# kepengxu/RealCamNet

Hardware: AMD Instinct MI355X
Metric: megapixels/sec RAW->sRGB at 4K (higher is better)
Workload: dtype bf16; 1 GPU; cfg3: 3840x2160 Bayer mosaic -> unshuffle+pad16 -> LiteISPNet_GFM_LSC_GMA -> sRGB 3840x2160, 8 frames/GPU, bf16 storage / fp32 accumulate; frames_per_gpu=8, global_frames=8, parallelism=frame-shard x1, collective=none

## Files before the change

### include/realcam_hip.h

```cpp
#ifndef REALCAM_HIP_H
#define REALCAM_HIP_H

#include <stddef.h>
#include <stdint.h>

#ifdef __cplusplus
extern "C" {
#endif

#define RC_ABI_VERSION 15

typedef enum rc_status {
    RC_OK = 0,
    RC_ERR_INVALID = -1,
    RC_ERR_HIP = -2,
    RC_ERR_UNSUPPORTED = -3
} rc_status;

typedef enum rc_dtype { RC_F32 = 0, RC_BF16 = 1, RC_U16 = 2 ,
                        RC_F16 = 3  } rc_dtype;

typedef enum rc_act { RC_ACT_NONE = 0, RC_ACT_RELU = 1, RC_ACT_LEAKY = 2 ,
                      RC_ACT_GELU = 3 ,
                      RC_ACT_RELU_POST = 4  } rc_act;

typedef enum rc_out_mode {
    RC_OUT_NHWC = 0,
    RC_OUT_PIXEL_SHUFFLE2 = 1,
    RC_OUT_NCHW = 2,
    RC_OUT_PIXEL_SHUFFLE2_NCHW = 3,
    RC_OUT_NHWC_DWT = 4
} rc_out_mode;

int rc_abi_version(void);
const char* rc_last_error(void);
const char* rc_build_info(void);
int rc_device_arch(char* buf, size_t buflen);

int rc_bayer_unshuffle(const void* d_mosaic, int in_dtype, void* d_packed, int out_dtype,
                       int batch, int h, int w, int hp, int wp, void* stream);

int rc_raw_ingest(const void* d_mosaic, int in_dtype, void* d_packed, void* d_cond, int out_dtype, int batch, int h, int w,
                  int hp, int wp, int cond_h, int cond_w, float black_level, float white_level, void* stream);

typedef enum rc_raw_storage {
    RC_RAW_F32 = 0, RC_RAW_BF16 = 1, RC_RAW_U16 = 2, RC_RAW_F16 = 3,
    RC_RAW_U8 = 4,
    RC_RAW_MIPI10 = 5,
    RC_RAW_MIPI12 = 6
} rc_raw_storage;

typedef enum rc_cfa { RC_CFA_RGGB = 0, RC_CFA_BGGR = 1, RC_CFA_GRBG = 2, RC_CFA_GBRG = 3 } rc_cfa;

typedef struct rc_raw_format {
    int storage;
    int cfa;
    int line_bytes;
    int width;
    float black[4];
    float white;
    int reserved[4];
} rc_raw_format;
size_t rc_raw_format_size(void);

int rc_raw_ingest_fmt(const void* d_src, const rc_raw_format* fmt, void* d_packed, void* d_cond, int out_dtype, int batch, int h, int w,
                      int hp, int wp, int cond_h, int cond_w, void* stream);

int rc_rgb_encode(const void* d_src, int src_dtype, void* d_dst, int out_bits, int batch, int H, int W, int h, int w, void* stream);

typedef enum rc_yuv_layout {
    RC_YUV_NV12 = 0,
    RC_YUV_P010 = 1,
    RC_YUV_I420 = 2
} rc_yuv_layout;
typedef enum rc_yuv_matrix { RC_MATRIX_BT601 = 0, RC_MATRIX_BT709 = 1, RC_MATRIX_BT2020 = 2  } rc_yuv_matrix;
typedef enum rc_yuv_range { RC_RANGE_LIMITED = 0, RC_RANGE_FULL = 1 } rc_yuv_range;
typedef enum rc_chroma_siting { RC_SITING_LEFT = 0 ,
                                RC_SITING_CENTER = 1  } rc_chroma_siting;

#define RC_YUV_KR_KB {{0.299, 0.114}, {0.2126, 0.0722}, {0.2627, 0.0593}}

typedef struct rc_out_format {
    int layout;
    int matrix;
    int range;
    int siting;
    int pitch;
    int rows;
    int chroma_offset[2];
    int reserved[4];
} rc_out_format;
size_t rc_out_format_size(void);

size_t rc_yuv_frame_bytes(const rc_out_format* fmt, int h, int w);

int rc_yuv_encode(const void* d_src, int src_dtype, const rc_out_format* fmt, void* d_dst, int batch, int H, int W, int h, int w, void* stream);

typedef enum rc_jpeg_subsampling { RC_JPEG_420 = 0 , RC_JPEG_444 = 1  } rc_jpeg_subsampling;

typedef struct rc_jpeg_desc {
    int quality;
    int subsampling;
    int restart;
    int reserved[5];
} rc_jpeg_desc;
size_t rc_jpeg_desc_size(void);

typedef struct rc_jpeg_plan_info {
    long long header_bytes;
    long long mcu_cols, mcu_rows;
    long long intervals;
    long long capacity;
    long long scratch_bytes;
} rc_jpeg_plan_info;
// ... 423 lines not shown
```

### realcamnet_amd/LiteISP.py

```python
from __future__ import annotations

from typing import Optional, Sequence

import torch
import torch.nn as nn

from . import networks as N
from . import ops
from .groupmix import GMA_Block, SUPPORTED_DTYPES
from ._lib import RC_OUT_NCHW, RC_OUT_PIXEL_SHUFFLE2
from .jpeg import Jpeg
from .out_format import OutFormat
from .stats import Stats
from .resize import Output


def color_block(in_filters, out_filters, normalization=False):
    layers = [N.Conv2d(in_filters, out_filters, 1, stride=1, padding=0),
              nn.AvgPool2d(3, stride=2, padding=1, count_include_pad=True),
              nn.LeakyReLU(0.2)]
    if normalization:
        layers.append(nn.InstanceNorm2d(out_filters, affine=True))
    return layers

# ... 346 lines not shown
    for o in outs:
        t = y if o.warp is None else ops.warp(y, o.warp)
        t = t if o.resize is None else ops.resize(t, o.resize)
        if o.tone is not None:
            t = ops.tone_map(t, o.tone)
        if o.look is not None:
            t = ops.lut3d(t, o.look)
        if o.sharpen is not None:
            t = ops.sharpen(t, o.sharpen)
        res.append(_encode(t, _out_bits(o.format)))
    return res


class _DwtUNet(nn.Module):

    output_dtype: Optional[torch.dtype] = None
    cond_from_raw = False

    def _build(self, ch_1, ch_2, ch_3, cond_c=None, lsc=False, nf=None, n_blocks=4):
        if cond_c is not None:
            self.classifier = Color_Condition_GFM(in_channels=4, out_c=cond_c)
        self.head = N.seq(N.conv(4, ch_1, mode='C'))
        if lsc:
            self.lsc = Lens_Shading_Correction(in_channels=2, out_c=ch_1, nf=ch_1)

        def gfm(i, c):
            if cond_c is not None:
                setattr(self, f"encoder_modulation{i}", N.seq(Res_GFM(in_nc=c, chan=c, cond_c=cond_c, out_nc=c, nf=nf[i - 1])))

        gfm(1, ch_1)
        self.down1 = N.seq(N.conv(ch_1, ch_1, mode='C'), N.RCAGroup(in_channels=ch_1, out_channels=ch_1, nb=n_blocks),
                           N.conv(ch_1, ch_1, mode='C'), N.DWTForward(ch_1))
        gfm(2, ch_1 * 4)
        self.down2 = N.seq(N.conv(ch_1 * 4, ch_1, mode='C'), N.RCAGroup(in_channels=ch_1, out_channels=ch_1, nb=n_blocks),
                           N.DWTForward(ch_1))
        gfm(3, ch_1 * 4)
        self.down3 = N.seq(N.conv(ch_1 * 4, ch_2, mode='C'), N.RCAGroup(in_channels=ch_2, out_channels=ch_2, nb=n_blocks),
                           N.DWTForward(ch_2))
        gfm(4, ch_2 * 4)
        self.middle = N.seq(N.conv(ch_2 * 4, ch_3, mode='C'), N.RCAGroup(in_channels=ch_3, out_channels=ch_3, nb=n_blocks),
                            N.RCAGroup(in_channels=ch_3, out_channels=ch_3, nb=n_blocks), N.conv(ch_3, ch_2 * 4, mode='C'))
        self.up3 = N.seq(N.DWTInverse(ch_2 * 4), N.RCAGroup(in_channels=ch_2, out_channels=ch_2, nb=n_blocks),
                         N.conv(ch_2, ch_1 * 4, mode='C'))
        self.up2 = N.seq(N.DWTInverse(ch_1 * 4), N.RCAGroup(in_channels=ch_1, out_channels=ch_1, nb=n_blocks),
                         N.conv(ch_1, ch_1 * 4, mode='C'))
        self.up1 = N.seq(N.DWTInverse(ch_1 * 4), N.RCAGroup(in_channels=ch_1, out_channels=ch_1, nb=n_blocks),
                         N.conv(ch_1, ch_1, mode='C'))
        self.tail = N.seq(N.conv(ch_1, ch_1 * 4, mode='C'), nn.PixelShuffle(upscale_factor=2), N.conv(ch_1, 3, mode='C'))

    def _act_dtype(self) -> torch.dtype:
        return self.head.weight.dtype

    def _refine_d1(self, d1):
        return d1

    def _check(self, raw):
        if self.training:
            raise RuntimeError("realcamnet_amd is an inference path: call .eval() first")
        if raw.dim() != 4 or raw.shape[1] != 4:
            raise ValueError(f"raw must be (B,4,H,W), got {tuple(raw.shape)}")
        if raw.shape[2] % 8 or raw.shape[3] % 8:
            raise ValueError(f"packed RAW H,W must be multiples of 8 (3 Haar levels), got {raw.shape[2]}x{raw.shape[3]}; "
                             "use forward_mosaic()/pad_to_multiple_of_16 for other sizes")

    def _front(self, a, cond, coord_nhwc):
        def head():
            if not hasattr(self, "lsc"):
                return self.head._nhwc(a)
            h = ops.lsc_chain(self.lsc, coord_nhwc, self.head, a)
            return h if h is not None else self.head._nhwc(a, mul_plus1=self.lsc._nhwc(coord_nhwc))

        if not hasattr(self, "classifier"):
            return head(), None
        cond = ops._req(cond, "cond")
        vec, h = ops.fork_join(lambda: self.classifier._vec(cond), head, [cond])
        return h, vec

    def _trunk(self, h, vec, crop_hw=None):
        mod = (lambda i, t: getattr(self, f"encoder_modulation{i}")._nhwc((t, vec))[0]) if vec is not None else (lambda i, t: t)
        h = mod(1, h)
        d1 = self._refine_d1(self.down1._nhwc(h))
        d2 = self.down2._nhwc(mod(2, d1))
        d3 = self.down3._nhwc(mod(3, d2))
        m = self.middle._nhwc(mod(4, d3), residual=d3)
        u3 = self.up3._nhwc(m, residual=d2)
        u2 = self.up2._nhwc(u3, residual=d1)
        u1 = self.up1._nhwc(u2, residual=h)
        if ops.tail_fold_ok(u1, self.tail[0], self.tail[2]):
            return ops.tail_fold(u1, self.tail[0], self.tail[2], crop_hw=crop_hw, out_dtype=self.output_dtype)
        t = self.tail[0]._nhwc(u1, out_mode=RC_OUT_PIXEL_SHUFFLE2)
        return self.tail[2]._nhwc(t, out_mode=RC_OUT_NCHW, crop_hw=crop_hw, out_dtype=self.output_dtype)

    def forward(self, x: Sequence[torch.Tensor]):
        raw = x if isinstance(x, torch.Tensor) else x[0]
        self._check(raw)
        dt = self._act_dtype()
        coord_nhwc = None
        if hasattr(self, "lsc"):
            coord = x[2]
            if coord.shape[0] != raw.shape[0] or coord.shape[1] != 2 or coord.shape[2:] != raw.shape[2:]:
                raise ValueError(f"coord must be (B,2,H,W) matching raw, got {tuple(coord.shape)}")
            coord_nhwc = ops.to_nhwc(coord, dtype=dt)
        cond = (raw if self.cond_from_raw else x[1]) if hasattr(self, "classifier") else None
        h, vec = self._front(ops.to_nhwc(raw, dtype=dt), cond, coord_nhwc)
        return self._trunk(h, vec)

    def forward_mosaic(self, mosaic, cond=None, coord=None, pad_to: int = 16, black_level: float = 0.0, white_level: float = 1.0,
                       cond_hw=(256, 256), raw_format=None, out_format=None, outputs=None):
        if self.training:
            raise RuntimeError("realcamnet_amd is an inference path: call .eval() first")
        bits = _out_bits(out_format)
        dt = self._act_dtype()
        mh, mw = _mosaic_hw(mosaic, raw_format)
        outs = _plan_outputs(outputs, out_format, (mh, mw))
        a, cond = _ingest(self, mosaic, cond, dt, pad_to, black_level, white_level, cond_hw, raw_format)
        b, hp, wp, _ = a.shape
        co = None
        if hasattr(self, "lsc"):
            if coord is None or coord.shape[-2:] != (mh // 2, mw // 2):
                raise ValueError("coord must be at packed resolution (h, w)")
            co = ops.to_nhwc(coord, dtype=dt, pad_hw=(hp, wp))
        if hasattr(self, "classifier") and self.cond_from_raw:
            cond = ops.to_nchw(a)
        h, vec = self._front(a, cond, co)
        return _emit(self._trunk(h, vec, crop_hw=(mh, mw)), bits, outs)


class LiteISPNet(_DwtUNet):

    def __init__(self):
        super().__init__()
        self._build(64, 128, 128)


class LiteISPNet_GFM_LSC(_DwtUNet):

    def __init__(self):
        super().__init__()
        self._build(48, 128, 128, cond_c=32, lsc=True, nf=(48, 48, 48, 128))


class LiteISPNet_LSC(_DwtUNet):

    def __init__(self):
        super().__init__()
        self._build(48, 128, 128, lsc=True)


class LiteISPNet_GFM(_DwtUNet):

    def __init__(self):
        super().__init__()
        self._build(64, 128, 128, cond_c=64, nf=(64, 64, 64, 128))


class LiteISPNet_GFMresize(_DwtUNet):
    cond_from_raw = True

    def __init__(self):
        super().__init__()
        self._build(64, 128, 128, cond_c=32, nf=(128, 256, 256, 512))


class _StridedUNet(nn.Module):

    output_dtype: Optional[torch.dtype] = None

    cond_from_raw = False
    coord_in_intro = False
    skips = True
# ... 270 lines not shown
```

### realcamnet_amd/_lib.py

```python
from __future__ import annotations

import ctypes as C
import os
import re
from pathlib import Path

PKG = Path(__file__).resolve().parent
LIB_PATH = Path(os.environ["RC_HIP_LIB"]) if os.environ.get("RC_HIP_LIB") else PKG / "librealcam_hip.so"
HEADER = PKG.parent / "include" / "realcam_hip.h"

RC_F32, RC_BF16, RC_U16, RC_F16 = 0, 1, 2, 3
RC_ACT_NONE, RC_ACT_RELU, RC_ACT_LEAKY, RC_ACT_GELU, RC_ACT_RELU_POST = 0, 1, 2, 3, 4
RC_OUT_NHWC, RC_OUT_PIXEL_SHUFFLE2, RC_OUT_NCHW, RC_OUT_PIXEL_SHUFFLE2_NCHW, RC_OUT_NHWC_DWT = 0, 1, 2, 3, 4
ABI_VERSION = 15
RC_RAW_F32, RC_RAW_BF16, RC_RAW_U16, RC_RAW_F16, RC_RAW_U8, RC_RAW_MIPI10, RC_RAW_MIPI12 = 0, 1, 2, 3, 4, 5, 6
RC_CFA_RGGB, RC_CFA_BGGR, RC_CFA_GRBG, RC_CFA_GBRG = 0, 1, 2, 3
RC_YUV_NV12, RC_YUV_P010, RC_YUV_I420 = 0, 1, 2
RC_MATRIX_BT601, RC_MATRIX_BT709, RC_MATRIX_BT2020 = 0, 1, 2
RC_RANGE_LIMITED, RC_RANGE_FULL = 0, 1
RC_SITING_LEFT, RC_SITING_CENTER = 0, 1
RC_JPEG_420, RC_JPEG_444 = 0, 1
RC_FILTER_AREA, RC_FILTER_BILINEAR = 0, 1
RC_RESIZE_MAX_TAPS, RC_RESIZE_MAX_RATIO = 20, 8
RC_LUT3D_MIN_SIZE, RC_LUT3D_MAX_SIZE = 2, 65
RC_WARP_BILINEAR, RC_WARP_BICUBIC = 0, 1
RC_WARP_CLAMP, RC_WARP_CONSTANT = 0, 1
RC_WARP_MIN_CELL_LOG2, RC_WARP_MAX_CELL_LOG2, RC_WARP_MAX_DIM = 3, 6, 1 << 23
RC_STATS_MAX_GRID, RC_STATS_SLOTS = 64, 8
RC_TONE_MAX_GRID, RC_TONE_BINS = 16, 256
RC_DEFECT_HOT, RC_DEFECT_COLD = 1, 2
RC_CALIB_GAINS, RC_CALIB_CLIP, RC_CALIB_MAX_KNOTS = 1, 2, 16
RC_HDR_MOTION = 1
RC_TNR_RESET, RC_TNR_GAIN = 1, 2
RC_QUAD_REMOSAIC, RC_QUAD_BIN = 0, 1


class ConvDesc(C.Structure):
    _fields_ = [
        ("batch", C.c_int32), ("height", C.c_int32), ("width", C.c_int32),
        ("cin", C.c_int32), ("cout", C.c_int32), ("ksize", C.c_int32),
        ("dtype", C.c_int32),
        ("in0", C.c_void_p), ("in1", C.c_void_p), ("in_gate", C.c_void_p), ("in_store", C.c_void_p),
        ("wpacked", C.c_void_p), ("bias", C.c_void_p),
        ("film_scale", C.c_void_p), ("film_shift", C.c_void_p),
        ("act", C.c_int32), ("act_slope", C.c_float),
        ("mul_plus1", C.c_void_p), ("residual", C.c_void_p),
        ("out", C.c_void_p), ("out_mode", C.c_int32), ("out_dtype", C.c_int32),
        ("out_h", C.c_int32), ("out_w", C.c_int32),
        ("chan_sums", C.c_void_p),
        ("src_h", C.c_int32), ("src_w", C.c_int32),
        ("out_scale", C.c_void_p),
        ("chan_sums_slots", C.c_int32), ("cout_tile", C.c_int32),
        ("algo", C.c_int32),
    ]


class ConvPairDesc(C.Structure):
    _fields_ = [
        ("batch", C.c_int32), ("height", C.c_int32), ("width", C.c_int32), ("channels", C.c_int32),
        ("dtype", C.c_int32),
        ("in0", C.c_void_p), ("in1", C.c_void_p), ("in_gate", C.c_void_p), ("in_store", C.c_void_p),
        ("w1", C.c_void_p), ("b1", C.c_void_p),
        ("film_scale", C.c_void_p), ("film_shift", C.c_void_p),
        ("act1", C.c_int32), ("act1_slope", C.c_float),
        ("w2", C.c_void_p), ("b2", C.c_void_p),
        ("residual", C.c_void_p), ("out", C.c_void_p), ("chan_sums", C.c_void_p),
    ]


class RawFormatDesc(C.Structure):
    _fields_ = [
        ("storage", C.c_int32), ("cfa", C.c_int32), ("line_bytes", C.c_int32), ("width", C.c_int32),
        ("black", C.c_float * 4), ("white", C.c_float), ("reserved", C.c_int32 * 4),
    ]


class OutFormatDesc(C.Structure):
    _fields_ = [
        ("layout", C.c_int32), ("matrix", C.c_int32), ("range", C.c_int32), ("siting", C.c_int32),
        ("pitch", C.c_int32), ("rows", C.c_int32), ("chroma_offset", C.c_int32 * 2), ("reserved", C.c_int32 * 4),
    ]


class JpegDesc(C.Structure):
    _fields_ = [("quality", C.c_int32), ("subsampling", C.c_int32), ("restart", C.c_int32), ("reserved", C.c_int32 * 5)]


class JpegPlanInfo(C.Structure):
    _fields_ = [("header_bytes", C.c_longlong), ("mcu_cols", C.c_longlong), ("mcu_rows", C.c_longlong), ("intervals", C.c_longlong),
                ("capacity", C.c_longlong), ("scratch_bytes", C.c_longlong)]


class StatsDesc(C.Structure):
    _fields_ = [
        ("roi", C.c_int32 * 4), ("grid", C.c_int32 * 2), ("bits", C.c_int32), ("matrix", C.c_int32), ("dark", C.c_int32), ("clip", C.c_int32),
        ("reserved", C.c_int32 * 4),
# ... 257 lines not shown
```

### realcamnet_amd/csrc/conv.hip

```cpp
#include <mutex>
#include <vector>

#include "conv32_kernel.hpp"

namespace rc {

struct ConvPlan {
    int ck = 0, nt = 0, unit = 0, upt = 0, nu = 0, steps = 0;
    int n_chunks = 0, n_ct = 0, cout_packed = 0;
    int m32 = 0;
};

static int g_persist_on = 1;
extern int g_dw3_seg16;
extern int g_dec_lds;
extern int g_wmsa_mfma;
extern int g_pw_grid_cap;
static int g_pss = 0;
static int g_poison = 0;
static int g_thin = 2;
static int g_auto = 1;
static int g_sums_compact = 1;
static int g_conv32 = 0;

// ... 235 lines not shown
    if (std::string(key) == "pair_impl") { g_pair_impl = value < 0 || value > 2 ? 0 : value; return RC_OK; }
    if (std::string(key) == "dec_lds") { g_dec_lds = value != 0; return RC_OK; }
    if (std::string(key) == "dw3_seg16") { g_dw3_seg16 = value != 0; return RC_OK; }
    if (std::string(key) == "wmsa_mfma") { g_wmsa_mfma = value != 0; return RC_OK; }
    if (std::string(key) == "pss") { g_pss = value != 0; return RC_OK; }
    if (std::string(key) == "sums_compact") { g_sums_compact = value != 0; return RC_OK; }
    if (std::string(key) == "persist_auto") { g_auto = value < 0 ? 0 : (value > 2 ? 2 : value); return RC_OK; }
    if (std::string(key) == "thin") { g_thin = value < 0 ? 0 : (value > 2 ? 2 : value); return RC_OK; }
    if (std::string(key) == "lds_poison") { g_poison = value != 0; return RC_OK; }
    if (std::string(key) == "conv32") { g_conv32 = value < 0 ? 0 : (value > 4 ? 4 : value); return RC_OK; }
    if (std::string(key) == "wino_nnt") { wino_set_nnt(value); return RC_OK; }
    if (std::string(key) == "pw_grid_cap") { g_pw_grid_cap = value <= 0 || value > (1 << 22) ? (1 << 22) : value; return RC_OK; }
    return fail(RC_ERR_INVALID, std::string("rc_debug_set: unknown key ") + key);
}

int rc_debug_get(const char* key) {
    if (key == nullptr) return -1;
    if (std::string(key) == "persist") return g_persist_on;
    if (std::string(key) == "conv32") return g_conv32;
    if (std::string(key) == "conv_flags") return g_dbg_flags;
    if (std::string(key) == "pss") return g_pss;
    if (std::string(key) == "sums_compact") return g_sums_compact;
    if (std::string(key) == "persist_auto") return g_auto;
    if (std::string(key) == "thin") return g_thin;
    if (std::string(key) == "lds_poison") return g_poison;
    if (std::string(key) == "wino_nnt") return wino_get_nnt();
    if (std::string(key) == "pw_grid_cap") return g_pw_grid_cap;
    return -1;
}

int rc_debug_set_ptr(const char* key, void* p) {
    RC_REQUIRE(key != nullptr, "rc_debug_set_ptr: null key");
    if (std::string(key) == "conv_phase_timing") { g_dbg_ptr = static_cast<long long*>(p); return RC_OK; }
    return fail(RC_ERR_INVALID, std::string("rc_debug_set_ptr: unknown key ") + key);
}

int rc_prof_enable(int on) {
    std::lock_guard<std::mutex> lk(g_prof_mu);
    for (auto& r : g_prof) { (void)hipEventDestroy(r.e0); (void)hipEventDestroy(r.e1); }
    g_prof.clear();
    g_prof_on = on != 0;
    return RC_OK;
}

int rc_prof_collect(int64_t* n_launches, double* total_ms, double* total_flops) {
    std::lock_guard<std::mutex> lk(g_prof_mu);
    double ms = 0.0, fl = 0.0;
    for (auto& r : g_prof) {
        RC_HIP_CHECK(hipEventSynchronize(r.e1));
        float t = 0.f;
        RC_HIP_CHECK(hipEventElapsedTime(&t, r.e0, r.e1));
        ms += t; fl += r.flops;
    }
    if (n_launches) *n_launches = (int64_t)g_prof.size();
    if (total_ms) *total_ms = ms;
    if (total_flops) *total_flops = fl;
    return RC_OK;
}

int rc_prof_collect_rows(rc_prof_row* rows, int max_rows, int* n_rows) {
    RC_REQUIRE(rows != nullptr && n_rows != nullptr && max_rows >= 1, "rc_prof_collect_rows: bad arguments");
    std::lock_guard<std::mutex> lk(g_prof_mu);
    int n = 0;
    for (auto& r : g_prof) {
        RC_HIP_CHECK(hipEventSynchronize(r.e1));
        float t = 0.f;
        RC_HIP_CHECK(hipEventElapsedTime(&t, r.e0, r.e1));
        int i = 0;
        while (i < n && !(rows[i].cin == r.cin && rows[i].cout == r.cout && rows[i].ksize == r.ksize)) ++i;
        if (i == n) {
            if (n == max_rows) continue;
            rows[n] = rc_prof_row{r.cin, r.cout, r.ksize, 0, 0.0, 0.0, 0.0};
            ++n;
        }
        rows[i].launches += 1; rows[i].ms += t; rows[i].flops += r.flops; rows[i].bytes += r.bytes;
    }
    *n_rows = n;
    return RC_OK;
}

static int conv_build_args(const rc_conv_desc* d, ConvPlan& p, ConvArgs& a, size_t& es_out) {
    RC_REQUIRE(d != nullptr, "rc_conv2d: null desc");
    const bool dwt = d->out_mode == RC_OUT_NHWC_DWT;
    RC_REQUIRE(make_plan(d->cin, d->cout, d->ksize, d->dtype, dwt ? (int)RC_OUT_NHWC : d->out_mode, &p, d->cout_tile), "rc_conv2d: unsupported cin/cout/ksize/dtype/cout_tile");
    RC_REQUIRE(d->batch >= 1 && d->height >= 1 && d->width >= 1, "rc_conv2d: empty tensor");
    RC_REQUIRE(d->batch <= 65535, "rc_conv2d: batch > 65535");
    RC_REQUIRE(d->in0 && d->wpacked && d->out, "rc_conv2d: null in0/wpacked/out");
    RC_REQUIRE(d->out_mode >= RC_OUT_NHWC && d->out_mode <= RC_OUT_NHWC_DWT, "rc_conv2d: bad out_mode");
    if (dwt) {
        RC_REQUIRE(d->height % 2 == 0 && d->width % 2 == 0, "rc_conv2d: RC_OUT_NHWC_DWT needs even height and width");
        RC_REQUIRE(d->out_dtype == d->dtype && reinterpret_cast<uintptr_t>(d->out) % 16 == 0, "rc_conv2d: RC_OUT_NHWC_DWT: out_dtype must equal dtype, out 16-byte aligned");
        RC_REQUIRE(!d->mul_plus1 && !d->film_scale && !d->out_scale && !d->chan_sums && !d->in_gate && !d->in1 && !d->in_store && !d->src_h && !d->src_w && !d->cout_tile,
                   "rc_conv2d: RC_OUT_NHWC_DWT excludes mul_plus1 / film / out_scale / chan_sums / gated input / src_h / cout_tile");
        if (d->dtype == RC_F32 || d->ksize != 3 || p.m32 || !(d->act == RC_ACT_NONE || ((d->act == RC_ACT_RELU || d->act == RC_ACT_LEAKY) && !d->residual)))
            return fail(RC_ERR_UNSUPPORTED, "rc_conv2d: RC_OUT_NHWC_DWT is a bf16 / fp16 3x3 form with act NONE / RELU / LEAKY, or act NONE + residual");
    }
    RC_REQUIRE(d->act >= RC_ACT_NONE && d->act <= RC_ACT_RELU_POST, "rc_conv2d: bad act");
    RC_REQUIRE(d->act != RC_ACT_RELU_POST || (d->residual != nullptr && d->mul_plus1 == nullptr && d->film_scale == nullptr && d->chan_sums == nullptr),
               "rc_conv2d: RC_ACT_RELU_POST is relu(conv + residual): needs residual, excludes film / mul_plus1 / chan_sums");
    if (d->in_gate) RC_REQUIRE(d->in1 != nullptr, "rc_conv2d: in_gate needs in1 (the skip tensor)");
    RC_REQUIRE((d->film_scale == nullptr) == (d->film_shift == nullptr), "rc_conv2d: film_scale/film_shift must come together");
    const bool full_tiles = d->cout == p.cout_packed;
    if (d->mul_plus1 || d->residual)
        RC_REQUIRE((full_tiles || d->cout % 4 == 0) && (d->out_mode == RC_OUT_NHWC || (dwt && !d->mul_plus1)), "rc_conv2d: mul_plus1/residual need cout % 4 == 0 and RC_OUT_NHWC (residual: or RC_OUT_NHWC_DWT)");
    if (d->chan_sums) RC_REQUIRE(d->out_mode == RC_OUT_NHWC, "rc_conv2d: chan_sums needs RC_OUT_NHWC");
    if (d->out_scale) {
        RC_REQUIRE(d->out_mode == RC_OUT_NHWC && !p.m32, "rc_conv2d: out_scale needs RC_OUT_NHWC and a layer outside the 32x32x16 forms");
        RC_REQUIRE(reinterpret_cast<uintptr_t>(d->out_scale) % 4 == 0, "rc_conv2d: out_scale must be 4-byte aligned");
    }
    const size_t es = dtype_size(d->dtype);
    const int planar16 = d->dtype == RC_F16 ? RC_F16 : RC_BF16;
    if (dwt) {
    } else if (d->out_mode == RC_OUT_NHWC) {
        RC_REQUIRE(d->out_dtype == d->dtype, "rc_conv2d: out_dtype must equal dtype for RC_OUT_NHWC");
        RC_REQUIRE(!full_tiles || (d->cout * es) % 8 == 0, "rc_conv2d: cout*elem_size must be a multiple of 8 bytes for RC_OUT_NHWC");
        RC_REQUIRE(reinterpret_cast<uintptr_t>(d->out) % 16 == 0, "rc_conv2d: out must be 16-byte aligned");
        if (p.nt == 4 && d->dtype != RC_F32) RC_REQUIRE(d->cout % 8 == 0, "rc_conv2d: cout % 8");
    } else if (d->out_mode == RC_OUT_PIXEL_SHUFFLE2) {
        RC_REQUIRE(d->out_dtype == d->dtype, "rc_conv2d: out_dtype must equal dtype for RC_OUT_PIXEL_SHUFFLE2");
        RC_REQUIRE(full_tiles && ((d->cout / 4) * es) % 8 == 0, "rc_conv2d: pixel-shuffle store needs (cout/4)*elem_size % 8 == 0");
        RC_REQUIRE(!d->film_scale, "rc_conv2d: film not supported with pixel-shuffle store");
        RC_REQUIRE(reinterpret_cast<uintptr_t>(d->out) % 16 == 0, "rc_conv2d: out must be 16-byte aligned");
    } else if (d->out_mode == RC_OUT_PIXEL_SHUFFLE2_NCHW) {
        RC_REQUIRE(d->out_h >= 1 && d->out_h <= 2 * d->height && d->out_w >= 1 && d->out_w <= 2 * d->width, "rc_conv2d: bad pixel-shuffle NCHW crop");
        RC_REQUIRE(d->out_dtype == RC_F32 || d->out_dtype == planar16, "rc_conv2d: bad out_dtype");
        RC_REQUIRE(!d->chan_sums, "rc_conv2d: chan_sums needs RC_OUT_NHWC");
        RC_REQUIRE((double)d->out_h * d->out_w * (d->cout / 4) * 4.0 < 2147483647.0, "rc_conv2d: one output image must be < 2 GiB");
    } else {
        RC_REQUIRE(d->out_h >= 1 && d->out_h <= d->height && d->out_w >= 1 && d->out_w <= d->width, "rc_conv2d: bad NCHW crop");
        RC_REQUIRE(d->out_dtype == RC_F32 || d->out_dtype == planar16, "rc_conv2d: bad out_dtype");
    }
    {
        const double lim = 2147483647.0;
        RC_REQUIRE((double)d->height * d->width * d->cin * es < lim, "rc_conv2d: one input image must be < 2 GiB");
        RC_REQUIRE((double)d->height * d->width * d->cout * 4.0 < lim, "rc_conv2d: one output image must be < 2 GiB");
    }
    const bool fold = d->src_h != 0 || d->src_w != 0;
    if (fold) {
        RC_REQUIRE(d->ksize == 2 && d->cin % 4 == 0 && (d->cin / 4) % p.ck == 0, "rc_conv2d: src_h/src_w need ksize 2 and cin / 4 a whole number of Cin chunks");
        RC_REQUIRE(d->src_h >= 1 && d->src_w >= 1 && d->height == (d->src_h + 1) / 2 && d->width == (d->src_w + 1) / 2,
                   "rc_conv2d: height/width must be ceil(src_h / 2), ceil(src_w / 2)");
        RC_REQUIRE(d->in_gate == nullptr && d->in1 == nullptr && d->in_store == nullptr, "rc_conv2d: src_h/src_w exclude the gated input");
        RC_REQUIRE(reinterpret_cast<uintptr_t>(d->in0) % 16 == 0, "rc_conv2d: src_h/src_w need a 16-byte aligned in0 (the scalar staging path does not gather)");
        RC_REQUIRE((double)d->src_h * d->src_w * (d->cin / 4) * es < 2147483647.0, "rc_conv2d: one input image must be < 2 GiB");
    }
    if (d->residual) RC_REQUIRE(reinterpret_cast<uintptr_t>(d->residual) % 16 == 0, "rc_conv2d: residual must be 16-byte aligned");
    if (d->mul_plus1) RC_REQUIRE(reinterpret_cast<uintptr_t>(d->mul_plus1) % 16 == 0, "rc_conv2d: mul_plus1 must be 16-byte aligned");

    a = ConvArgs{};
    a.batch = d->batch; a.H = d->height; a.W = d->width; a.cin = d->cin; a.cout = d->cout;
    a.n_chunks = p.n_chunks; a.n_ct = p.n_ct;
    a.tiles_x = ceil_div(d->width, kTW); a.tiles_y = ceil_div(d->height, kTH);
    if (p.m32) RC_REQUIRE(!d->film_scale || (reinterpret_cast<uintptr_t>(d->film_scale) % 16 == 0 && reinterpret_cast<uintptr_t>(d->film_shift) % 16 == 0),
                          "rc_conv2d: film vectors must be 16-byte aligned");
    auto aligned16 = [](const void* q) { return q == nullptr || reinterpret_cast<uintptr_t>(q) % 16 == 0; };
    a.cin_vec_ok = (d->cin % p.unit == 0) && aligned16(d->in0) && aligned16(d->in1) && aligned16(d->in_store) &&
                   (d->in_gate == nullptr || reinterpret_cast<uintptr_t>(d->in_gate) % 4 == 0);
    a.cin_chunk_ok = d->cin % p.ck == 0;
    a.fold2 = fold ? 1 : 0; a.src_H = d->src_h; a.src_W = d->src_w; a.cfold = d->cin / 4;
    a.in0 = d->in0; a.in1 = d->in1; a.in_gate = d->in_gate; a.in_store = d->in_store;
    a.wpacked = d->wpacked; a.bias = d->bias;
    a.film_scale = d->film_scale; a.film_shift = d->film_shift;
    a.act = d->act; a.act_slope = d->act_slope;
    a.mul_plus1 = d->mul_plus1; a.residual = d->residual; a.out_scale = d->out_scale;
    a.out = d->out; a.out_mode = d->out_mode; a.out_dtype = d->out_dtype; a.out_h = d->out_h; a.out_w = d->out_w;
    a.chan_sums = d->chan_sums; a.cout_packed = p.cout_packed;
    a.sum_slots = d->chan_sums_slots > 0 ? d->chan_sums_slots : 4 * ceil_div(d->height, kTH) * ceil_div(d->width, kTW);
    a.sums_compact = 0; a.query = nullptr; a.sums_compact_ok = g_sums_compact;
    {
        int key = (d->act == RC_ACT_RELU ? 1 : 0) | (d->act == RC_ACT_LEAKY ? 2 : 0) | (d->film_scale ? 4 : 0) |
                  (d->mul_plus1 ? 8 : 0) | (d->residual ? 16 : 0) | (d->chan_sums ? 32 : 0) | (d->out_scale ? 64 : 0);
        bool fast = full_tiles && d->out_mode != RC_OUT_NCHW && d->out_mode != RC_OUT_PIXEL_SHUFFLE2_NCHW && d->act != RC_ACT_GELU && d->act != RC_ACT_RELU_POST;
        if (d->act == RC_ACT_LEAKY) fast = fast && d->act_slope >= 0.f && d->act_slope <= 1.f;
        if (d->film_scale)
            fast = fast && d->cout % 4 == 0 && reinterpret_cast<uintptr_t>(d->film_scale) % 16 == 0 && reinterpret_cast<uintptr_t>(d->film_shift) % 16 == 0;
        if (d->out_scale) fast = fast && d->cout % 4 == 0 && reinterpret_cast<uintptr_t>(d->out_scale) % 16 == 0;
        switch (key) { case 0: case 1: case 2: case 16: case 32: case 8: case 6: case 33: case 34: case 80: break; default: fast = false; }
        a.ep_key = fast ? key : -1;
        a.pss = g_pss && d->out_mode == RC_OUT_PIXEL_SHUFFLE2 && !p.m32 && p.n_chunks == 1 && p.n_ct == 4 && d->cout == 4 * 16 * p.nt &&
                d->dtype == RC_BF16 && d->in_gate == nullptr && fast && (key == 0 || key == 1 || key == 2);
    }
    {
        const int num_cus = device_cu_count();
        a.num_cus = num_cus;
        a.persist_ok = g_persist_on;
        a.auto_impl = g_auto;
        a.thin = g_thin;
        a.dbg = g_dbg_ptr;
        a.dbg_flags = g_dbg_flags;
        a.td = make_tile_decode(a.tiles_x, a.tiles_y, kBandRows);
        a.td_wsm = make_tile_decode(a.tiles_x, (a.H + kWsmTH - 1) / kWsmTH, kBandRows);
        a.div_n_ct = make_magic(a.n_ct);
    }
    es_out = es;
    return RC_OK;
// ... 44 lines not shown
```

### realcamnet_amd/csrc/conv_kernel.hpp

```cpp
#pragma once
#include "common.hpp"

namespace rc {

struct MagicDiv { unsigned m, sh; };
inline MagicDiv make_magic(int d) {
    if (d <= 1) return MagicDiv{0u, 0u};
    int L = 0;
    while ((2 << L) <= d) ++L;
    const unsigned long long m = ((1ull << (31 + L)) + (unsigned long long)d - 1) / (unsigned long long)d;
    return MagicDiv{(unsigned)m, (unsigned)(L - 1)};
}
__device__ __forceinline__ int magic_div(int n, const MagicDiv& d) {
    return d.m ? (int)(__umulhi((unsigned)n, d.m) >> d.sh) : n;
}
struct TileDecode { MagicDiv sp_total, band, last_rows; };
inline TileDecode make_tile_decode(int tiles_x, int tiles_y, int band_rows) {
    return TileDecode{make_magic(tiles_x * tiles_y), make_magic(band_rows * tiles_x), make_magic(tiles_y % band_rows ? tiles_y % band_rows : 1)};
}

struct ConvArgs {
    int batch, H, W, cin, cout;
    int n_chunks, n_ct, tiles_x, tiles_y;
    int cin_vec_ok;
// ... 822 lines not shown
            if constexpr ((F & EP_SUMS) != 0) {
#pragma unroll
                for (int e = 0; e < NV; ++e) run[e] += valid ? v[e] : 0.f;
            }
            const int oo = (valid && !(a.dbg_flags & 1)) ? (((gy + p) * a.W + gx) * a.cout + jbase) * ES : kOOB;
            buf_store_row<T, NV, PK_RELU>(r_out, oo, v);
        }
        if constexpr ((F & EP_SUMS) != 0) {
            if (flush) {
                write_chan_sums(a, b, slot, n, jbase, run, false);
#pragma unroll
                for (int e = 0; e < NV; ++e) run[e] = 0.f;
            }
        }
    }

    template <int F>
    __device__ static __forceinline__ void epilogue_dwt(const ConvArgs& a, int b, int y0, int x0, int tid, f32x4 (&acc)[4][NT], char* st,
                                                        const unsigned (&rp)[(F & EP_RES) ? 4 : 1][(F & EP_RES) ? NV / 2 : 1]) {
        static_assert(ES == 2 && NV % 4 == 0 && (F == 0 || F == EP_RELU || F == EP_LEAKY || F == EP_RES), "bf16; plain / ReLU / LeakyReLU / + residual");
        typedef float f32x2 __attribute__((ext_vector_type(2)));
        const int lane = tid & 63, wave = tid >> 6, q = lane >> 4, n = lane & 15;
        constexpr int REC = Cfg::COUT_TILE * 2 + 8, ROW = kTW * REC;
        const float inf = __builtin_inff();
#pragma unroll
        for (int pt = 0; pt < 4; ++pt) {
            float v[NV];
#pragma unroll
            for (int nt = 0; nt < NT; ++nt)
#pragma unroll
                for (int r = 0; r < 4; ++r) v[nt * 4 + r] = acc[pt][nt][r];
            if constexpr ((F & EP_RELU) != 0) {
#pragma unroll
                for (int e = 0; e < NV; ++e) v[e] = __builtin_amdgcn_fmed3f(v[e], 0.f, inf);
            }
            if constexpr ((F & EP_LEAKY) != 0) {
#pragma unroll
                for (int e = 0; e < NV; ++e) v[e] = __builtin_amdgcn_fmed3f(v[e], v[e] * a.act_slope, inf);
            }
            if constexpr ((F & EP_RES) != 0) {
#pragma unroll
                for (int i = 0; i < NV / 2; ++i) {
                    v[2 * i] += lo16<T>(rp[pt][i]);
                    v[2 * i + 1] += hi16<T>(rp[pt][i]);
                }
            }
            char* dst = st + (pt >> 1) * ROW + (16 * (pt & 1) + n) * REC + q * (NV * 2);
#pragma unroll
            for (int i = 0; i < NV / 4; ++i)
                *reinterpret_cast<uint2*>(dst + 8 * i) = make_uint2(pack16x2<T>(v[4 * i], v[4 * i + 1]), pack16x2<T>(v[4 * i + 2], v[4 * i + 3]));
        }
        __builtin_amdgcn_fence(__ATOMIC_RELEASE, "wavefront");
        __builtin_amdgcn_wave_barrier();
        f32x2 in[4][NV / 2];
        const char* src = st + (2 * n) * REC + q * (NV * 2);
#pragma unroll
        for (int t = 0; t < 4; ++t)
#pragma unroll
            for (int i = 0; i < NV / 4; ++i) {
                const uint2 w = *reinterpret_cast<const uint2*>(src + (t >> 1) * ROW + (t & 1) * REC + 8 * i);
                in[t][2 * i] = f32x2{lo16<T>(w.x), hi16<T>(w.x)} * 0.5f;
                in[t][2 * i + 1] = f32x2{lo16<T>(w.y), hi16<T>(w.y)} * 0.5f;
            }
        __builtin_amdgcn_fence(__ATOMIC_RELEASE, "wavefront");
        __builtin_amdgcn_wave_barrier();
        unsigned o[2 * NV];
#pragma unroll
        for (int p = 0; p < NV / 2; ++p) {
            const f32x2 sab = in[0][p] + in[1][p], dab = in[0][p] - in[1][p];
            const f32x2 k0 = (sab + in[2][p]) + in[3][p], k1 = (sab - in[2][p]) - in[3][p];
            const f32x2 k2 = (dab + in[2][p]) - in[3][p], k3 = (dab - in[2][p]) + in[3][p];
            o[4 * p] = pack16x2<T>(k0.x, k1.x); o[4 * p + 1] = pack16x2<T>(k2.x, k3.x);
            o[4 * p + 2] = pack16x2<T>(k0.y, k1.y); o[4 * p + 3] = pack16x2<T>(k2.y, k3.y);
        }
        const int Hh = a.H >> 1, Wh = a.W >> 1, oy = (y0 >> 1) + wave, ox = (x0 >> 1) + n;
        const size_t img_out = (size_t)a.H * a.W * a.cout;
        const __amdgpu_buffer_rsrc_t r_out = make_rsrc(static_cast<T*>(a.out) + (size_t)b * img_out, (unsigned)(img_out * ES));
        const int oo = (oy < Hh && ox < Wh && !(a.dbg_flags & 1)) ? ((oy * Wh + ox) * (4 * a.cout) + 4 * q * NV) * ES : kOOB;
#pragma unroll
        for (int i = 0; i < NV / 2; ++i)
            __builtin_amdgcn_raw_buffer_store_b128(u32x4_t{o[4 * i], o[4 * i + 1], o[4 * i + 2], o[4 * i + 3]}, r_out, oo, 16 * i, 0);
    }

    __device__ static __forceinline__ void epilogue_generic(const ConvArgs& a, int b, int y0, int x0, int sp, int ct, int tid,
                                                            f32x4 (&acc)[4][NT]) {
        const int lane = tid & 63, wave = tid >> 6, q = lane >> 4, n = lane & 15;
        const int jbase = ct * Cfg::COUT_TILE + q * NV;
        float fs[NV], ft[NV];
        const bool film = a.film_scale != nullptr;
        if (film) {
#pragma unroll
            for (int e = 0; e < NV; ++e) {
                const bool in = jbase + e < a.cout;
                fs[e] = in ? a.film_scale[(size_t)b * a.cout + jbase + e] : 0.f;
                ft[e] = in ? a.film_shift[(size_t)b * a.cout + jbase + e] : 0.f;
            }
        }
        const int gy_w = y0 + 2 * wave, gx_l = x0 + n;
        float csum[NV];
#pragma unroll
        for (int e = 0; e < NV; ++e) csum[e] = 0.f;

        const size_t img_out = (size_t)a.H * a.W * a.cout;
        const unsigned img_bytes_out = (unsigned)(img_out * ES);
        __amdgpu_buffer_rsrc_t r_out;
        if (a.out_mode == RC_OUT_NCHW || a.out_mode == RC_OUT_PIXEL_SHUFFLE2_NCHW) {
            const size_t plane = (size_t)a.out_h * a.out_w;
            const int osz = a.out_dtype == RC_F32 ? 4 : 2;
            const int planes = a.out_mode == RC_OUT_NCHW ? a.cout : a.cout >> 2;
            r_out = make_rsrc(static_cast<char*>(a.out) + (size_t)b * planes * plane * osz, (unsigned)(planes * plane * osz));
        } else {
            r_out = make_rsrc(static_cast<T*>(a.out) + (size_t)b * img_out, img_bytes_out);
        }
        const bool full = a.cout == a.cout_packed;

#pragma unroll
        for (int pt = 0; pt < 4; ++pt) {
            const int gy = gy_w + (pt >> 1);
            const int gx = gx_l + (pt & 1) * 16;
            const bool valid = gy < a.H && gx < a.W;
            float v[NV];
#pragma unroll
            for (int nt = 0; nt < NT; ++nt)
#pragma unroll
                for (int r = 0; r < 4; ++r) v[nt * 4 + r] = acc[pt][nt][r];
            if (film) {
#pragma unroll
                for (int e = 0; e < NV; ++e) v[e] = v[e] * fs[e] + ft[e] + v[e];
            }
            if (a.act == RC_ACT_RELU) {
#pragma unroll
                for (int e = 0; e < NV; ++e) v[e] = __builtin_amdgcn_fmed3f(v[e], 0.f, __builtin_inff());
            } else if (a.act == RC_ACT_LEAKY) {
#pragma unroll
                for (int e = 0; e < NV; ++e) v[e] = v[e] > 0.f ? v[e] : v[e] * a.act_slope;
            } else if (a.act == RC_ACT_GELU) {
#pragma unroll
                for (int e = 0; e < NV; ++e) v[e] = gelu_erf_f32(v[e]);
            }
            const int pix_off = valid ? ((gy * a.W + gx) * a.cout + jbase) * ES : kOOB;
            if (a.mul_plus1 != nullptr) {
                float m[NV];
                const __amdgpu_buffer_rsrc_t r_mul = make_rsrc(static_cast<const T*>(a.mul_plus1) + (size_t)b * img_out, img_bytes_out);
                buf_load_row<T, NV>(r_mul, pix_off, m);
#pragma unroll
                for (int e = 0; e < NV; ++e) v[e] = v[e] * (m[e] + 1.f);
            }
            if (a.out_scale != nullptr) {
#pragma unroll
                for (int e = 0; e < NV; ++e) v[e] *= (jbase + e < a.cout) ? a.out_scale[(size_t)b * a.cout + jbase + e] : 0.f;
            }
            if (a.residual != nullptr) {
                float m[NV];
                const __amdgpu_buffer_rsrc_t r_res = make_rsrc(static_cast<const T*>(a.residual) + (size_t)b * img_out, img_bytes_out);
                buf_load_row<T, NV>(r_res, pix_off, m);
#pragma unroll
                for (int e = 0; e < NV; ++e) v[e] += m[e];
                if (a.act == RC_ACT_RELU_POST) {
#pragma unroll
                    for (int e = 0; e < NV; ++e) v[e] = __builtin_amdgcn_fmed3f(v[e], 0.f, __builtin_inff());
                }
            }
            if (a.chan_sums != nullptr) {
#pragma unroll
                for (int e = 0; e < NV; ++e) csum[e] += valid ? v[e] : 0.f;
            }
// ... 58 lines not shown

template <class Cfg, bool GATED, bool FAST>
__global__ __launch_bounds__(kThreads, 2) void conv_mfma_kernel(const ConvArgs a) {
    using D = ConvDev<Cfg>;
    using T = typename Cfg::elem;
    constexpr int NT = Cfg::NT, STEPS = Cfg::STEPS, G = Cfg::G, NSUB = Cfg::NSUB, NV = 4 * NT;

    extern __shared__ __attribute__((aligned(16))) char smem[];
    char* s_w = smem;
    char* s_in = smem + Cfg::W_BYTES;

    const int tid = threadIdx.x, lane = tid & 63, wave = tid >> 6;
    const int q = lane >> 4, n = lane & 15;
    const int ct = blockIdx.x % a.n_ct;
    const int sp = blockIdx.x / a.n_ct;
    const int tx = sp % a.tiles_x, ty = sp / a.tiles_x;
    const int b = blockIdx.y;
    const int y0 = ty * kTH, x0 = tx * kTW;

    typename D::LaneOff lo;
    D::lane_offsets(q, lo);
    const int lane_x = ((2 * wave) * D::TWH + n) * D::SPIX;
    const int lane_w = lane * 16;

    f32x4 acc[4][NT];
#pragma unroll
    for (int nt = 0; nt < NT; ++nt) {
        f32x4 bv = f32x4{0.f, 0.f, 0.f, 0.f};
        if (a.bias) {
            const float4 t4 = *reinterpret_cast<const float4*>(a.bias + ct * Cfg::COUT_TILE + q * NV + nt * 4);
            bv = f32x4{t4.x, t4.y, t4.z, t4.w};
        }
#pragma unroll
        for (int pt = 0; pt < 4; ++pt) acc[pt][nt] = bv;
    }

    ConvArgs aa = a;
    if (ct != 0) aa.in_store = nullptr;
    const typename D::TileSrc ts = D::tile_src(aa, b, y0, x0);
    typename D::TileOffs to;
    D::tile_offsets(aa, tid, to);
    const char* wbase = static_cast<const char*>(a.wpacked) + (size_t)ct * a.n_chunks * Cfg::CHUNK_W_BYTES;

    for (int chunk = 0; chunk < a.n_chunks; ++chunk) {
        if (chunk > 0) __syncthreads();
        const char* wchunk = wbase + (size_t)chunk * Cfg::CHUNK_W_BYTES;
        D::dma_weights(wchunk, s_w, (STEPS < G ? STEPS : G) * NT, wave, lane_w);
        if (a.cin_vec_ok) {
            uint4 r0[D::NI], r1[GATED ? D::NI : 1];
            float gv[GATED ? D::UNIT : 1];
            D::template load_tile<GATED>(aa, ts, to, b, chunk, tid, r0, r1, gv);
            D::template commit_tile<GATED>(aa, ts, to, chunk, tid, r0, r1, gv, s_in);
        } else {
            D::stage_tile_scalar(aa, b, y0, x0, chunk, tid, s_in, static_cast<T*>(aa.in_store));
        }
        __syncthreads();
        D::template mma_steps<0, G, 0>(s_in, s_w, lane_x, lane_w, q, lo, acc);
        if constexpr (NSUB > 1) {
            __syncthreads();
            D::dma_weights(wchunk + (size_t)G * NT * 1024, s_w, ((STEPS - G) < G ? (STEPS - G) : G) * NT, wave, lane_w);
            __syncthreads();
            D::template mma_steps<G, G, G>(s_in, s_w, lane_x, lane_w, q, lo, acc);
        }
        if constexpr (NSUB > 2) {
            __syncthreads();
            D::dma_weights(wchunk + (size_t)2 * G * NT * 1024, s_w, ((STEPS - 2 * G) < G ? (STEPS - 2 * G) : G) * NT, wave, lane_w);
            __syncthreads();
            D::template mma_steps<2 * G, G, 2 * G>(s_in, s_w, lane_x, lane_w, q, lo, acc);
        }
        static_assert(NSUB <= 3, "add another weight sub-stage");
    }
    D::template epilogue<FAST>(a, b, y0, x0, sp, ct, tid, acc);
}

constexpr int kPersistMaxCout = 512;
template <class Cfg>
constexpr int persist_bias_slots() { return Cfg::KS == 5 ? 64 : kPersistMaxCout; }
template <class Cfg>
constexpr int persist_lds_bytes_c() { return Cfg::IN_BYTES + (int)Cfg::CHUNK_W_BYTES + persist_bias_slots<Cfg>() * 4; }

template <class Cfg>
constexpr int persist_blocks_per_cu() { return Cfg::NT <= 2 && persist_lds_bytes_c<Cfg>() * 3 <= 160 * 1024 ? 3 : 2; }

template <class Cfg, bool GATED, bool FAST>
__global__ __launch_bounds__(kThreads, persist_blocks_per_cu<Cfg>()) void conv_mfma_persist_kernel(const ConvArgs a) {
    using D = ConvDev<Cfg>;
    constexpr int NT = Cfg::NT, STEPS = Cfg::STEPS, NV = 4 * NT;

    const int w_copies = a.w_resident ? a.n_ct : 1;
    extern __shared__ __attribute__((aligned(16))) char smem[];
    char* s_w = smem;
    float* s_bias = reinterpret_cast<float*>(smem + w_copies * Cfg::CHUNK_W_BYTES);
    char* s_in = smem + w_copies * Cfg::CHUNK_W_BYTES + persist_bias_slots<Cfg>() * 4;

    const int tid = threadIdx.x, lane = tid & 63, wave = tid >> 6;
    const int q = lane >> 4, n = lane & 15;
    typename D::LaneOff lo;
    D::lane_offsets(q, lo);
    const int lane_x = ((2 * wave) * D::TWH + n) * D::SPIX;
    const int lane_w = lane * 16;

    const int sp_total = a.tiles_x * a.tiles_y;
    const int n_tiles = sp_total * a.batch;
    const int n_ct = a.n_ct;
    const int slots = gridDim.x >> 3;
    const int pos = (blockIdx.x & 7) * slots + (blockIdx.x >> 3);

    if (n_ct == 1 || a.w_resident) D::dma_weights(static_cast<const char*>(a.wpacked), s_w, STEPS * NT * w_copies, wave, lane_w);
    for (int i = tid; i < a.cout_packed; i += kThreads) s_bias[i] = a.bias ? a.bias[i] : 0.f;

    uint4 r0[D::NI], r1[GATED ? D::NI : 1];
    float gv[GATED ? D::UNIT : 1];
    typename D::TileOffs to;
    D::tile_offsets(a, tid, to);
    int tile = pos < n_tiles ? pos : -1;
    int b = 0, sp = 0, y0 = 0, x0 = 0;
    typename D::TileSrc ts;
    if (tile >= 0) {
        b = magic_div(tile, a.td.sp_total);
        int ty, tx;
        band_decode(tile - b * sp_total, a.tiles_x, a.tiles_y, a.td, ty, tx);
        sp = ty * a.tiles_x + tx; y0 = ty * kTH; x0 = tx * kTW;
        ts = D::tile_src(a, b, y0, x0);
        if (a.cin_vec_ok) {
            D::template load_gate<GATED>(a, b, 0, tid, gv);
            if (ts.interior) D::template load_tile_interior<GATED>(a, ts, to, 0, r0, r1);
        }
    }
    float run[NV];
#pragma unroll
    for (int e = 0; e < NV; ++e) run[e] = 0.f;
    int covered = 0;
    constexpr bool BORDER_PRE = !GATED && Cfg::KS == 3 && (NT == 3 || NT == 4) && sizeof(typename Cfg::elem) == 2;
    bool first_tile = true;
    while (tile >= 0) {
        __syncthreads();
        if (a.cin_vec_ok && !ts.interior && (!BORDER_PRE || first_tile || (a.dbg_flags & 16))) D::template load_tile_border<GATED>(a, ts, 0, tid, r0, r1);
        first_tile = false;
        if (a.cin_vec_ok) D::template commit_tile<GATED>(a, ts, to, 0, tid, r0, r1, gv, s_in);
        else D::stage_tile_scalar(a, b, y0, x0, 0, tid, s_in, static_cast<typename Cfg::elem*>(a.in_store));
        constexpr bool RUN_SUMS = FAST && sizeof(typename Cfg::elem) == 2 && NT >= 3;
        const int cb = b, csp = sp, cy0 = y0, cx0 = x0;
        const int next = tile + (int)gridDim.x;
        tile = next < n_tiles ? next : -1;
        if constexpr (RUN_SUMS) {
            const bool will_flush = tile < 0 || magic_div(tile, a.td.sp_total) != cb;
            if ((a.ep_key == D::EP_SUMS || a.ep_key == (D::EP_RELU | D::EP_SUMS)) && n_ct == 1) {
                if (!a.sums_compact) { if (!will_flush) D::zero_sum_slots(a, cb, csp, tid); }
                else if (will_flush) {
                    for (int bb = covered; bb < cb; ++bb) D::zero_slots4(a, bb, 4 * D::compact_residue(pos, bb, sp_total, (int)gridDim.x), tid);
                    covered = cb + 1;
                }
            }
        }

        for (int ct = 0; ct < n_ct; ++ct) {
            if (n_ct > 1 && !a.w_resident) {
                if (ct > 0) __syncthreads();
                D::dma_weights(static_cast<const char*>(a.wpacked) + (size_t)ct * Cfg::CHUNK_W_BYTES, s_w, STEPS * NT, wave, lane_w);
            }
            if (ct == 0 || !a.w_resident) __syncthreads();
            if (ct == n_ct - 1 && tile >= 0) {
                b = magic_div(tile, a.td.sp_total);
                int ty, tx;
                band_decode(tile - b * sp_total, a.tiles_x, a.tiles_y, a.td, ty, tx);
                sp = ty * a.tiles_x + tx; y0 = ty * kTH; x0 = tx * kTW;
                ts = D::tile_src(a, b, y0, x0);
                if (a.cin_vec_ok) {
                    D::template load_gate<GATED>(a, b, 0, tid, gv);
                    if (ts.interior) D::template load_tile_interior<GATED>(a, ts, to, 0, r0, r1);
                    else if constexpr (BORDER_PRE) { if (!(a.dbg_flags & 16)) D::template load_tile_border<GATED>(a, ts, 0, tid, r0, r1); }
                }
            }
            f32x4 acc[4][NT];
#pragma unroll
            for (int nt = 0; nt < NT; ++nt) {
                const float4 t4 = *reinterpret_cast<const float4*>(s_bias + ct * Cfg::COUT_TILE + q * NV + nt * 4);
#pragma unroll
                for (int pt = 0; pt < 4; ++pt) acc[pt][nt] = f32x4{t4.x, t4.y, t4.z, t4.w};
            }
            constexpr bool RESPRE = FAST && !GATED && sizeof(typename Cfg::elem) == 2 && NT <= 3;
            [[maybe_unused]] unsigned rpre[RESPRE ? 4 : 1][RESPRE ? D::NRH : 1];
            bool res_pre = false;
            if constexpr (RESPRE) {
                if ((a.ep_key == D::EP_RES || a.ep_key == (D::EP_GATE | D::EP_RES)) && a.out_mode == RC_OUT_NHWC) {
                    res_pre = true;
                    D::res_prefetch(a, cb, cy0, cx0, ct, tid, rpre);
                }
            }
            D::template mma_steps<0, STEPS, 0, (!GATED && NT < 5)>(s_in, a.w_resident ? s_w + ct * (int)Cfg::CHUNK_W_BYTES : s_w, lane_x, lane_w, q, lo, acc);
            if constexpr (FAST && sizeof(typename Cfg::elem) == 2) {
                const int rslot = a.sums_compact ? 4 * D::compact_residue(pos, cb, sp_total, (int)gridDim.x) : -1;
                if (RUN_SUMS && a.ep_key == D::EP_SUMS && n_ct == 1)
                    D::template epilogue_fast_impl<D::EP_SUMS, RUN_SUMS>(a, cb, cy0, cx0, csp, ct, tid, acc, run, tile < 0 || b != cb, rslot);
                else if (RUN_SUMS && a.ep_key == (D::EP_RELU | D::EP_SUMS) && n_ct == 1)
                    D::template epilogue_fast_impl<D::EP_RELU | D::EP_SUMS, RUN_SUMS>(a, cb, cy0, cx0, csp, ct, tid, acc, run, tile < 0 || b != cb, rslot);
                else if (res_pre) {
                    if constexpr (RESPRE) {
                        D::epilogue_res_pre(a, cb, cy0, cx0, ct, tid, acc, rpre, a.ep_key == (D::EP_GATE | D::EP_RES) ? a.out_scale + (size_t)cb * a.cout : nullptr);
                    }
                } else D::template epilogue<FAST>(a, cb, cy0, cx0, csp, ct, tid, acc);
            } else D::template epilogue<FAST>(a, cb, cy0, cx0, csp, ct, tid, acc);
        }
    }
    if constexpr (FAST && sizeof(typename Cfg::elem) == 2 && NT >= 3) {
        if (a.sums_compact && (a.ep_key == D::EP_SUMS || a.ep_key == (D::EP_RELU | D::EP_SUMS)) && n_ct == 1)
            for (int bb = covered; bb < a.batch; ++bb) D::zero_slots4(a, bb, 4 * D::compact_residue(pos, bb, sp_total, (int)gridDim.x), tid);
    }
}

constexpr int kWsThreads = 512;

template <class Cfg, bool GATED, bool FAST>
__global__ __launch_bounds__(kWsThreads) void conv_mfma_ws_kernel(const ConvArgs a) {
    using D = ConvDev<Cfg>;
    constexpr int NT = Cfg::NT, STEPS = Cfg::STEPS, NV = 4 * NT;

    extern __shared__ __attribute__((aligned(16))) char smem[];
    char* s_w = smem;
    float* s_bias = reinterpret_cast<float*>(smem + Cfg::CHUNK_W_BYTES);
    char* s_buf0 = smem + Cfg::CHUNK_W_BYTES + 16 * Cfg::NT * 4;
    char* s_buf1 = s_buf0 + Cfg::IN_BYTES;

    const int tid = threadIdx.x, lane = tid & 63;
    const int wave8 = __builtin_amdgcn_readfirstlane(tid >> 6);
    const bool loader = wave8 >= 4;
    const int rtid = tid & 255, wave = wave8 & 3;
    const int q = lane >> 4, n = lane & 15;

    const int sp_total = a.tiles_x * a.tiles_y;
    const int n_tiles = sp_total * a.batch;
    const int slots = gridDim.x >> 3;
    const int pos = (blockIdx.x & 7) * slots + (blockIdx.x >> 3);
    const int stride = (int)gridDim.x;
    const int my_tiles = pos < n_tiles ? (n_tiles - pos + stride - 1) / stride : 0;

    for (int kb = wave8; kb < STEPS * NT; kb += kWsThreads / 64)
        __builtin_amdgcn_global_load_lds((const __attribute__((address_space(1))) void*)(static_cast<const char*>(a.wpacked) + kb * 1024 + lane * 16),
                                         (__attribute__((address_space(3))) void*)(s_w + kb * 1024), 16, 0, 0);
    for (int i = tid; i < a.cout_packed; i += kWsThreads) s_bias[i] = a.bias ? a.bias[i] : 0.f;

    auto decode = [&](int tile, int& b, int& sp, int& y0, int& x0) {
        b = magic_div(tile, a.td.sp_total);
        int ty, tx;
        band_decode(tile - b * sp_total, a.tiles_x, a.tiles_y, a.td, ty, tx);
        sp = ty * a.tiles_x + tx; y0 = ty * kTH; x0 = tx * kTW;
    };

    if (loader) {
        uint4 r0[D::NI], r1[GATED ? D::NI : 1];
        float gv[GATED ? D::UNIT : 1];
        typename D::TileSrc ts;
        typename D::TileOffs to;
        D::tile_offsets(a, rtid, to);
        int b, sp, y0, x0;
        if (my_tiles > 0) {
            decode(pos, b, sp, y0, x0);
            ts = D::tile_src(a, b, y0, x0);
            D::template load_tile<GATED>(a, ts, to, b, 0, rtid, r0, r1, gv);
            D::template commit_tile<GATED>(a, ts, to, 0, rtid, r0, r1, gv, s_buf0);
        }
        if (my_tiles > 1) {
            decode(pos + stride, b, sp, y0, x0);
            ts = D::tile_src(a, b, y0, x0);
            D::template load_tile<GATED>(a, ts, to, b, 0, rtid, r0, r1, gv);
        }
        __syncthreads();
        const bool rec = a.dbg != nullptr && blockIdx.x == 8 && wave8 == 4 && lane == 0;
        for (int k = 0; k < my_tiles; ++k) {
            const long long tl0 = rec ? (long long)__builtin_amdgcn_s_memtime() : 0;
            if (k + 1 < my_tiles) {
                D::template commit_tile<GATED>(a, ts, to, 0, rtid, r0, r1, gv, ((k + 1) & 1) ? s_buf1 : s_buf0);
                if (k + 2 < my_tiles) {
                    decode(pos + (k + 2) * stride, b, sp, y0, x0);
// ... 128 lines not shown
        __syncthreads();
        for (int g = 0; g < my_stages; ++g) {
            const int wsoff_g = wsoff;
            dma(WA, WB, wsoff_g);
            if (g + 1 < my_stages) issue_a();
            __syncthreads();
            if (g + 1 < my_stages) {
                if (need_wa()) dma(0, WA, wsoff);
                commit_a();
            }
            __syncthreads();
        }
    } else {
        const int wave = wave12;
        typename D::LaneOff lo;
        D::lane_offsets(q, lo);
        const int lane_x = ((2 * wave) * D::TWH + n) * D::SPIX;
        const int lane_w = lane * 16;
        __syncthreads();
        int g = 0;
        for (int k = 0; k < my_units; ++k) {
            int b, ty, tx, ct0;
            decode(pos + k * stride, b, ty, tx, ct0);
            const int ty8 = 2 * ty + (wave >> 2);
            for (int ct = ct0; ct < ct0 + cts_per_unit; ++ct) {
                f32x4 acc[4][NT];
#pragma unroll
                for (int nt = 0; nt < NT; ++nt) {
                    const float4 t4 = *reinterpret_cast<const float4*>(s_bias + ct * Cfg::COUT_TILE + q * NV + nt * 4);
#pragma unroll
                    for (int pt = 0; pt < 4; ++pt) acc[pt][nt] = f32x4{t4.x, t4.y, t4.z, t4.w};
                }
                auto run_chunks = [&](auto PH, int c0, int c1) {
                    constexpr int ph = decltype(PH)::value;
                    for (int c = c0; c < c1; ++c, ++g) {
                        const char* s_in = s_in0 + (one_chunk ? (k & 1) : (g & 1)) * Cfg::IN_BYTES;
                        if constexpr (ph == 3) { if (!(a.dbg_flags & 2)) D::template mma_steps<0, SA, 0, true>(s_in, s_w, lane_x, lane_w, q, lo, acc); }
                        else if constexpr (ph == 2) D::template mma_steps<1, 1, 0, false>(s_in, s_w, lane_x, lane_w, q, lo, acc);
                        __syncthreads();
                        if constexpr ((ph & 1) != 0) { if (!(a.dbg_flags & 2)) D::template mma_steps<SA, STEPS - SA, 0, true>(s_in, s_w, lane_x, lane_w, q, lo, acc); }
                        else D::template mma_steps<3, 1, 0, false>(s_in, s_w, lane_x, lane_w, q, lo, acc);
                        if (c + 1 < n_chunks) __syncthreads();
                    }
                };
                if constexpr (FOLD_SKIP) {
                    const int cpp = D::folded(a) ? n_chunks >> 2 : 0;
                    run_chunks(std::integral_constant<int, 0>{}, 0, cpp);
                    run_chunks(std::integral_constant<int, 1>{}, cpp, 2 * cpp);
                    run_chunks(std::integral_constant<int, 2>{}, 2 * cpp, 3 * cpp);
                    run_chunks(std::integral_constant<int, 3>{}, 3 * cpp, n_chunks);
                } else {
                    run_chunks(std::integral_constant<int, 3>{}, 0, n_chunks);
                }
                if (ty8 < a.tiles_y)
                    D8::template epilogue<FAST>(a, b, ty8 * kTH, tx * kTW, ty8 * a.tiles_x + tx, ct, tid & 255, acc);
                __syncthreads();
            }
        }
    }
}

template <class Cfg8>
struct WstCfg : WsmCfg<Cfg8> {
    using B = WsmCfg<Cfg8>;
    static constexpr int SPIX = B::CK * (int)sizeof(typename B::elem);
    static constexpr int N_PIECES = B::THH * B::TWH * B::UPT;
    static constexpr int N_DMA = (N_PIECES + 63) / 64;
    static constexpr int IN_BYTES = N_DMA * 1024;
};
template <class Cfg>
constexpr int wst_form() {
    if (!(sizeof(typename Cfg::elem) == 2 && (Cfg::KS == 2 || Cfg::KS == 3) && (Cfg::UPT == 2 || Cfg::UPT == 4) && Cfg::STEPS >= 2)) return 0;
    const int w = (int)Cfg::CHUNK_W_BYTES, in = WstCfg<Cfg>::IN_BYTES, fixed = 2 * w + kPersistMaxCout * 4;
    if (w <= 20 * 1024 && fixed + 3 * in <= 160 * 1024) return 3;
    if (w <= 36 * 1024 && fixed + 2 * in <= 160 * 1024) return 2;
    return 0;
}
template <class Cfg>
constexpr int wst_lds_bytes() { return 2 * (int)Cfg::CHUNK_W_BYTES + kPersistMaxCout * 4 + (wst_form<Cfg>() == 3 ? 3 : 2) * WstCfg<Cfg>::IN_BYTES; }
template <class Cfg>
constexpr bool wst_eligible() { return wst_form<Cfg>() != 0; }
constexpr int waitcnt_vm(int n) { return (n & 15) | ((n >> 4) << 14) | 0x0F70; }

template <class Cfg8, bool FAST>
__global__ __launch_bounds__(kWsmThreads) void conv_mfma_wst_kernel(const ConvArgs a) {
#if defined(__HIP_DEVICE_COMPILE__)
    using Cfg = WstCfg<Cfg8>;
    using D = ConvDev<Cfg>;
    using D8 = ConvDev<Cfg8>;
    constexpr int NT = Cfg::NT, STEPS = Cfg::STEPS, NV = 4 * NT, WALL = (int)Cfg::CHUNK_W_BYTES, UPT = Cfg::UPT, TWH = Cfg::TWH, ES = 2;
    constexpr int N_DMA = Cfg::N_DMA, NDW = (N_DMA + 3) / 4;
    constexpr int NBUF = wst_form<Cfg8>() == 3 ? 3 : 2;
    constexpr bool FOLD_SKIP = Cfg::KS == 2 && UPT == 4 && STEPS == 4;

    extern __shared__ __attribute__((aligned(16))) char smem[];
    char* s_w = smem;
    float* s_bias = reinterpret_cast<float*>(smem + 2 * WALL);
    char* s_in0 = smem + 2 * WALL + kPersistMaxCout * 4;

    const int tid = threadIdx.x, lane = tid & 63;
    const int wave12 = __builtin_amdgcn_readfirstlane(tid >> 6);
    const bool loader = wave12 >= 8;
    const int q = lane >> 4, n = lane & 15;

    const int tiles_y = (a.H + kWsmTH - 1) / kWsmTH;
    const int sp_total = a.tiles_x * tiles_y;
    const int n_tiles = sp_total * a.batch;
    const int n_chunks = a.n_chunks, n_ct = a.n_ct;
    const bool one_chunk = n_chunks == 1;
    const int n_units = one_chunk ? n_tiles : n_tiles * n_ct;
    const int cts_per_unit = one_chunk ? n_ct : 1;
    const int slots = gridDim.x >> 3;
    const int pos = (blockIdx.x & 7) * slots + (blockIdx.x >> 3);
    const int stride = (int)gridDim.x;
    const int my_units = pos < n_units ? (n_units - pos + stride - 1) / stride : 0;
    const int my_stages = my_units * cts_per_unit * n_chunks;

    for (int i = tid; i < a.cout_packed; i += kWsmThreads) s_bias[i] = a.bias ? a.bias[i] : 0.f;

    auto decode = [&](int unit, int& b, int& ty, int& tx, int& ct0) {
        int tile = unit;
        ct0 = 0;
        if (!one_chunk) { tile = magic_div(unit, a.div_n_ct); ct0 = unit - tile * n_ct; }
        b = magic_div(tile, a.td_wsm.sp_total);
        band_decode(tile - b * sp_total, a.tiles_x, tiles_y, a.td_wsm, ty, tx);
    };

    if (loader && NBUF == 2) {
        if constexpr (NBUF == 2) {
            const int rtid = tid - kWsmCompute, w4 = wave12 - 8;
            uint4 r0[D::NI], r1[1];
            float gv[1];
            typename D::TileSrc ts;
            typename D::TileOffs to;
            D::tile_offsets(a, rtid, to);
            int k_unit = 0, cti = 0, chunk = 0, gi = 0, ct = 0;
            int b = 0, ty = 0, tx = 0, ct0 = 0;
            auto fetch = [&]() {
                if (gi < my_stages) {
                    if (chunk == 0) {
                        if (cti == 0) decode(pos + k_unit * stride, b, ty, tx, ct0);
                        ct = ct0 + cti;
                        ts = D::tile_src(a, b, ty * kWsmTH, tx * kTW);
                    }
                    const int goff = (ct * n_chunks + chunk) * WALL;
                    for (int kb = w4; kb < WALL / 1024; kb += 4)
                        __builtin_amdgcn_global_load_lds((const __attribute__((address_space(1))) void*)(static_cast<const char*>(a.wpacked) + goff + kb * 1024 + lane * 16),
                                                         (__attribute__((address_space(3))) void*)(s_w + (gi & 1) * WALL + kb * 1024), 16, 0, 0);
                    if (!one_chunk || cti == 0) {
                        D::template load_tile<false>(a, ts, to, b, chunk, rtid, r0, r1, gv);
                        D::template commit_tile<false>(a, ts, to, chunk, rtid, r0, r1, gv, s_in0 + (one_chunk ? (k_unit & 1) : (gi & 1)) * Cfg::IN_BYTES);
                    }
                }
                ++gi;
                if (++chunk == n_chunks) { chunk = 0; if (++cti == cts_per_unit) { cti = 0; ++k_unit; } }
            };
            fetch();
            __syncthreads();
            for (int g = 0; g < my_stages; ++g) {
                fetch();
                __syncthreads();
            }
        }
    } else if (loader) {
        const int w4 = wave12 - 8;
        int lc[NDW];
#pragma unroll
// ... 36 lines not shown
                    }
                }
            }
            ++gi; gb3 = gb3 == 2 ? 0 : gb3 + 1;
            if (++chunk == n_chunks) { chunk = 0; if (++cti == cts_per_unit) { cti = 0; ++k_unit; kb3 = kb3 == 2 ? 0 : kb3 + 1; } }
            return in_flight;
        };
        int wi = 0, wk = 0, wcti = 0, wchunk = 0, wct0 = 0;
        auto issue_w = [&]() {
            if (wi < my_stages) {
                if (wchunk == 0 && wcti == 0) { int b_, ty_, tx_; decode(pos + wk * stride, b_, ty_, tx_, wct0); }
                const int goff = ((wct0 + wcti) * n_chunks + wchunk) * WALL;
                int ph = 3;
                if constexpr (FOLD_SKIP) ph = D::folded(a) ? D::fold_phase(a, wchunk * Cfg::CK) : 3;
                for (int kb = w4; kb < WALL / 1024; kb += 4) {
                    if constexpr (FOLD_SKIP) {
                        const int st = kb / NT;
                        if (!(st == 3 || ph == 3 || (ph == 1 && st == 2) || (ph == 2 && st == 1))) continue;
                    }
                    __builtin_amdgcn_global_load_lds((const __attribute__((address_space(1))) void*)(static_cast<const char*>(a.wpacked) + goff + kb * 1024 + lane * 16),
                                                     (__attribute__((address_space(3))) void*)(s_w + (wi & 1) * WALL + kb * 1024), 16, 0, 0);
                }
            }
            ++wi;
            if (++wchunk == n_chunks) { wchunk = 0; if (++wcti == cts_per_unit) { wcti = 0; ++wk; } }
        };
        issue_w();
        issue();
        issue();
        __syncthreads();
        for (int g = 0; g < my_stages; ++g) {
            issue_w();
            const int nfl = issue();
            if (nfl == NDW) __builtin_amdgcn_s_waitcnt(waitcnt_vm(NDW));
            else if (NDW > 1 && nfl == NDW - 1) __builtin_amdgcn_s_waitcnt(waitcnt_vm(NDW > 1 ? NDW - 1 : 0));
            else __builtin_amdgcn_s_waitcnt(waitcnt_vm(0));
            __builtin_amdgcn_s_barrier();
        }
        __builtin_amdgcn_s_waitcnt(waitcnt_vm(0));
    } else {
        const int wave = wave12;
        typename D::LaneOff lo;
        D::lane_offsets(q, lo);
        const int lane_x = ((2 * wave) * D::TWH + n) * D::SPIX;
        const int lane_w = lane * 16;
        __syncthreads();
        int g = 0, gb3 = 0, kb3 = 0;
        for (int k = 0; k < my_units; ++k) {
            int b, ty, tx, ct0;
            decode(pos + k * stride, b, ty, tx, ct0);
            const int ty8 = 2 * ty + (wave >> 2);
            for (int ct = ct0; ct < ct0 + cts_per_unit; ++ct) {
                f32x4 acc[4][NT];
#pragma unroll
                for (int nt = 0; nt < NT; ++nt) {
                    const float4 t4 = *reinterpret_cast<const float4*>(s_bias + ct * Cfg::COUT_TILE + q * NV + nt * 4);
#pragma unroll
                    for (int pt = 0; pt < 4; ++pt) acc[pt][nt] = f32x4{t4.x, t4.y, t4.z, t4.w};
                }
                auto run_chunks = [&](auto PH, int c0, int c1) {
                    constexpr int ph = decltype(PH)::value;
                    for (int c = c0; c < c1; ++c, ++g) {
                        const char* s_in = s_in0 + (one_chunk ? kb3 : gb3) * Cfg::IN_BYTES;
                        const char* s_wg = s_w + (g & 1) * WALL;
                        if constexpr (ph == 3) D::template mma_steps<0, STEPS, 0, true>(s_in, s_wg, lane_x, lane_w, q, lo, acc);
                        else if constexpr (ph == 1) D::template mma_steps<2, 2, 0, true>(s_in, s_wg, lane_x, lane_w, q, lo, acc);
                        else {
                            if constexpr (ph == 2) D::template mma_steps<1, 1, 0, false>(s_in, s_wg, lane_x, lane_w, q, lo, acc);
                            D::template mma_steps<3, 1, 0, false>(s_in, s_wg, lane_x, lane_w, q, lo, acc);
                        }
                        gb3 = gb3 == NBUF - 1 ? 0 : gb3 + 1;
                        if (c + 1 < n_chunks) __syncthreads();
                    }
                };
                if constexpr (FOLD_SKIP) {
                    const int cpp = D::folded(a) ? n_chunks >> 2 : 0;
                    run_chunks(std::integral_constant<int, 0>{}, 0, cpp);
                    run_chunks(std::integral_constant<int, 1>{}, cpp, 2 * cpp);
                    run_chunks(std::integral_constant<int, 2>{}, 2 * cpp, 3 * cpp);
                    run_chunks(std::integral_constant<int, 3>{}, 3 * cpp, n_chunks);
                } else {
                    run_chunks(std::integral_constant<int, 3>{}, 0, n_chunks);
                }
                if (ty8 < a.tiles_y)
                    D8::template epilogue<FAST>(a, b, ty8 * kTH, tx * kTW, ty8 * a.tiles_x + tx, ct, tid & 255, acc);
                __syncthreads();
            }
            kb3 = kb3 == NBUF - 1 ? 0 : kb3 + 1;
        }
    }
#endif
}

template <class Cfg>
constexpr int pss_lds_bytes() { return (int)Cfg::CHUNK_W_BYTES + kPersistMaxCout * 4 + WsmCfg<Cfg>::IN_BYTES + kWsmTH * kTW * Cfg::COUT_TILE * 2; }

template <class Cfg8>
__global__ __launch_bounds__(kWsmThreads) void conv_mfma_pss_kernel(const ConvArgs a) {
    using Cfg = WsmCfg<Cfg8>;
    using D = ConvDev<Cfg>;
    using T = typename Cfg::elem;
    static_assert(sizeof(T) == 2, "bf16 form");
    constexpr int NT = Cfg::NT, STEPS = Cfg::STEPS, NV = 4 * NT, NH = NV / 2;
    constexpr int SA = (STEPS + 1) / 2;
    constexpr int WA = SA * NT * 1024, WB = (STEPS - SA) * NT * 1024, WALL = (int)Cfg::CHUNK_W_BYTES;
    constexpr int NWA = (WA / 16 + kThreads - 1) / kThreads, NWB = (WB / 16 + kThreads - 1) / kThreads;
    constexpr int PXB = Cfg::COUT_TILE * 2, ROWB = kTW * PXB, OUTB = kWsmTH * ROWB;
    constexpr int UPP = PXB / 16, UPR = kTW * UPP;
    constexpr int NDR = OUTB / 16 / kThreads;
    static_assert(STEPS >= 2 && WA + WB == WALL && OUTB % (16 * kThreads) == 0 && NDR % 2 == 0 && PXB % 16 == 0, "pss shapes");

    extern __shared__ __attribute__((aligned(16))) char smem[];
    char* s_w = smem;
    float* s_bias = reinterpret_cast<float*>(smem + WALL);
    char* s_in = smem + WALL + kPersistMaxCout * 4;
    char* s_out = s_in + Cfg::IN_BYTES;

    const int tid = threadIdx.x, lane = tid & 63;
    const int wave12 = __builtin_amdgcn_readfirstlane(tid >> 6);
    const bool loader = wave12 >= 8;
    const int q = lane >> 4, n = lane & 15;

    const int tiles_y = (a.H + kWsmTH - 1) / kWsmTH;
    const int sp_total = a.tiles_x * tiles_y;
    const int n_tiles = sp_total * a.batch;
    constexpr int n_ct = 4;
    const int slots = gridDim.x >> 3;
    const int pos = (blockIdx.x & 7) * slots + (blockIdx.x >> 3);
    const int stride = (int)gridDim.x;
    const int my_units = pos < n_tiles ? (n_tiles - pos + stride - 1) / stride : 0;
    const int my_stages = my_units * n_ct;
    const int cps = a.cout >> 2;

    for (int i = tid; i < a.cout_packed; i += kWsmThreads) s_bias[i] = a.bias ? a.bias[i] : 0.f;

    auto decode = [&](int unit, int& b, int& ty, int& tx) {
        b = magic_div(unit, a.td_wsm.sp_total);
        band_decode(unit - b * sp_total, a.tiles_x, tiles_y, a.td_wsm, ty, tx);
    };

    if (loader) {
        const int rtid = tid - kWsmCompute;
        uint4 r0[D::NI], r1[1], wra[NWA], wrb[NWB];
        float gv[1];
        typename D::TileSrc ts;
        typename D::TileOffs to;
        D::tile_offsets(a, rtid, to);
        int lt = rtid;
        auto woa = [&](int k) { return (k * kThreads + lt) * 16 < WA ? (k * kThreads + lt) * 16 : kOOB; };
        auto wob = [&](int k) { return (k * kThreads + lt) * 16 < WB ? WA + (k * kThreads + lt) * 16 : kOOB; };
        const __amdgpu_buffer_rsrc_t r_w = make_rsrc(a.wpacked, (unsigned)((size_t)n_ct * WALL));
        const size_t img_out = (size_t)a.H * a.W * a.cout;

        int b = 0, ty = 0, tx = 0;
        int d_b = 0, d_y0 = 0, d_x0 = 0, d_ct = 0;
        int wsoff = 0;
        auto issue_tile = [&](int k) {
            decode(pos + k * stride, b, ty, tx);
            ts = D::tile_src(a, b, ty * kWsmTH, tx * kTW);
            D::template load_tile<false>(a, ts, to, b, 0, rtid, r0, r1, gv);
        };
        auto issue_wa = [&](int ct) {
            wsoff = ct * WALL;
#pragma unroll
            for (int k = 0; k < NWA; ++k) wra[k] = buf_load16(r_w, woa(k), wsoff);
        };
        auto issue_wb = [&]() {
#pragma unroll
// ... 385 lines not shown
    for (int e = 0; e < (MODE == 1 ? NV : 1); ++e) run[e] = 0.f;
    [[maybe_unused]] int covered = 0;

    while (cu_ >= 0) {
#pragma unroll
        for (int k = 0; k < NI; ++k) {
            const int row0 = (8 * k) / TWH, thr = (row0 + 1) * TWH - 8 * k;
            const int pix = 8 * k + j8;
            const int px = pix - TWH * (row0 + ((thr < 8 && j8 >= thr) ? 1 : 0));
            *reinterpret_cast<uint4*>(s_my + pix * kA64PXB + ((cu ^ (px & 7)) * 16)) = r[k];
        }
        const int gy = cty8 * kTH + 2 * wv, gx0 = ctx * kTW + 16 * chalf, sp = cty8 * a.tiles_x + ctx;
        int nb = cb, nty8 = cty8, ntx = ctx, nu = cu_;
        const int nhalf = chalf ^ 1;
        if (chalf == 1) nu = decode(cu_ + stride, nb, nty8, ntx);
        unsigned rpre[MODE == 2 ? 2 : 1][MODE == 2 ? D::NRH : 1];
        if constexpr (MODE == 2) D::sub_res_prefetch(a, cb, gy, gx0, lane, rpre);
        issue(nu >= 0, nb, nty8, ntx, nhalf);

        f32x4 acc[2][NT];
#pragma unroll
        for (int nt = 0; nt < NT; ++nt) {
            const float4 t4 = *reinterpret_cast<const float4*>(s_bias + q * NV + nt * 4);
            acc[0][nt] = f32x4{t4.x, t4.y, t4.z, t4.w};
            acc[1][nt] = f32x4{t4.x, t4.y, t4.z, t4.w};
        }
        if (!(a.dbg_flags & 2)) {
            uint4 wfa[NT], xfa[2], wfb[NT], xfb[2];
#pragma unroll
            for (int nt = 0; nt < NT; ++nt) wfa[nt] = *reinterpret_cast<const uint4*>(s_w + nt * 1024 + lane_w);
            xfa[0] = *reinterpret_cast<const uint4*>(s_my + xo[0][0]);
            xfa[1] = *reinterpret_cast<const uint4*>(s_my + xo[0][0] + kA64ROWB);
#pragma unroll
            for (int s = 0; s < STEPS; s += 2) {
                a64_step<T, 0, true, NT>(s, s_my, s_w, lane_w, xo, wfa, xfa, wfb, xfb, acc);
                if (s + 2 < STEPS) a64_step<T, 0, true, NT>(s + 1, s_my, s_w, lane_w, xo, wfb, xfb, wfa, xfa, acc);
                else a64_step<T, 0, false, NT>(s + 1, s_my, s_w, lane_w, xo, wfb, xfb, wfa, xfa, acc);
            }
        }

        if constexpr (MODE == 1) {
            const bool last = chalf == 1;
            const bool flush = last && (nu < 0 || nb != cb);
            int slot = 4 * sp + wv;
            if (!a.sums_compact) {
                if (last && !flush) D::zero_slot1(a, cb, slot, lane);
            } else if (flush) {
                for (int bb = covered; bb < cb; ++bb) D::zero_slot1(a, bb, 4 * D::compact_residue(pos, bb, sp_total, stride) + wv, lane);
                covered = cb + 1;
                slot = 4 * D::compact_residue(pos, cb, sp_total, stride) + wv;
            }
            const unsigned none[1][1] = {{0u}};
            if (a.ep_key == EP_SUMS) D::template epilogue_sub<EP_SUMS, 1>(a, cb, gy, gx0, slot, lane, acc, run, flush, none, nullptr);
            else if (a.ep_key == (EP_RELU | EP_SUMS)) D::template epilogue_sub<EP_RELU | EP_SUMS, 1>(a, cb, gy, gx0, slot, lane, acc, run, flush, none, nullptr);
            else D::template epilogue_sub<EP_LEAKY | EP_SUMS, 1>(a, cb, gy, gx0, slot, lane, acc, run, flush, none, nullptr);
        } else if constexpr (MODE == 2) {
            float none[1] = {0.f};
            if (gated_out) D::template epilogue_sub<EP_GATE | EP_RES, 2>(a, cb, gy, gx0, 0, lane, acc, none, false, rpre, s_gate + cb * a.cout);
            else D::template epilogue_sub<EP_RES, 2>(a, cb, gy, gx0, 0, lane, acc, none, false, rpre, nullptr);
        } else {
            float none[1] = {0.f};
            const unsigned nonr[1][1] = {{0u}};
            if (a.ep_key == EP_RELU) D::template epilogue_sub<EP_RELU, 1>(a, cb, gy, gx0, 0, lane, acc, none, false, nonr, nullptr);
            else if (a.ep_key == EP_LEAKY) D::template epilogue_sub<EP_LEAKY, 1>(a, cb, gy, gx0, 0, lane, acc, none, false, nonr, nullptr);
            else D::template epilogue_sub<0, 1>(a, cb, gy, gx0, 0, lane, acc, none, false, nonr, nullptr);
        }
        cu_ = nu; cb = nb; cty8 = nty8; ctx = ntx; chalf = nhalf;
    }
    if constexpr (MODE == 1) {
        if (a.sums_compact)
            for (int bb = covered; bb < a.batch; ++bb) D::zero_slot1(a, bb, 4 * D::compact_residue(pos, bb, sp_total, stride) + wv, lane);
    }
}

template <class Cfg>
constexpr int ws_lds_bytes() { return 2 * Cfg::IN_BYTES + (int)Cfg::CHUNK_W_BYTES + 16 * Cfg::NT * 4; }

template <class Cfg>
constexpr int persist_lds_bytes() { return persist_lds_bytes_c<Cfg>(); }

template <class Cfg, bool FAST>
int launch_wst(const ConvArgs& a, int grid, hipStream_t stream) {
    return launch_lds<&conv_mfma_wst_kernel<Cfg, FAST>>(dim3((unsigned)grid), dim3(kWsmThreads), wst_lds_bytes<Cfg>(), stream, a);
}

template <class Cfg, bool GATED, bool FAST>
int launch_conv_g(const ConvArgs& a, hipStream_t stream) {
    constexpr int P_LDS = persist_lds_bytes<Cfg>();
    constexpr bool P_OK = P_LDS <= 80 * 1024;
    const int n_tiles = a.tiles_x * a.tiles_y * a.batch;
    const int legacy_slots = 4 * a.tiles_x * a.tiles_y;
    auto report = [&](int kind, int slots) -> bool {
        if (a.query == nullptr) return false;
        a.query[0] = kind; a.query[1] = slots;
        return true;
    };
    auto sums_mode = [&](int compact_slots, int& compact) -> int {
        compact = 0;
        if (a.chan_sums == nullptr || a.sum_slots == legacy_slots) return RC_OK;
        if (compact_slots > 0 && a.sum_slots == compact_slots) { compact = 1; return RC_OK; }
        return fail(RC_ERR_INVALID, "rc_conv2d: chan_sums_slots matches neither layout of the kernel this launch takes (ask rc_conv_sum_slots)");
    };
    if (a.out_mode == RC_OUT_NHWC_DWT) {
        if constexpr (!GATED && FAST && auto_eligible<Cfg>()) {
            using DD = ConvDev<Cfg>;
            static_assert(StripCfg<Cfg>::IN_BYTES >= 2 * kTW * (Cfg::COUT_TILE * 2 + 8), "the strip's output fits its own halo strip");
            if ((a.ep_key == 0 || a.ep_key == DD::EP_RELU || a.ep_key == DD::EP_LEAKY || a.ep_key == DD::EP_RES) && a.n_chunks == 1 && a.n_ct == 1 && a.cout == Cfg::COUT_TILE &&
                a.cin_vec_ok && a.cin_chunk_ok && n_tiles < (1 << 24)) {
                if (report(0, legacy_slots)) return RC_OK;
                constexpr int A_LDS = auto_lds_bytes<Cfg>();
                const int n_items = a.tiles_x * ((a.H + kWsmTH - 1) / kWsmTH) * a.batch;
                const dim3 grid((unsigned)persistent_grid(a.num_cus, n_items));
                if (a.ep_key == DD::EP_RES) return launch_lds<&conv_mfma_auto_kernel<Cfg, 2>>(grid, dim3(kAutoThreads), A_LDS, stream, a);
                return launch_lds<&conv_mfma_auto_kernel<Cfg, 0>>(grid, dim3(kAutoThreads), A_LDS, stream, a);
            }
        }
        return fail(RC_ERR_UNSUPPORTED, "rc_conv2d: RC_OUT_NHWC_DWT needs a bf16 / fp16 3x3 layer of one Cin chunk and one 32- or 48-wide cout tile (cin == cout == 32 or 48), 16-byte aligned operands");
    }
    constexpr int WS_LDS = ws_lds_bytes<Cfg>();
    if constexpr (WS_LDS <= 150 * 1024) {
        const bool ws_auto = GATED || Cfg::NT == 5 || Cfg::CK == 80;
        if (a.n_chunks == 1 && a.n_ct == 1 && a.cin_vec_ok && (a.persist_ok == 2 || (a.persist_ok == 1 && ws_auto)) && n_tiles < (1 << 24)) {
            if (report(0, legacy_slots)) return RC_OK;
            { int c_; if (int e_ = sums_mode(0, c_)) return e_; }
            return launch_lds<&conv_mfma_ws_kernel<Cfg, GATED, FAST>>(dim3((unsigned)persistent_grid(a.num_cus, n_tiles)), dim3(kWsThreads), WS_LDS, stream, a);
        }
    }
    if constexpr (!GATED && FAST && dtype_of<typename Cfg::elem>::value == RC_BF16 && Cfg::KS == 3 && Cfg::STEPS >= 2 && pss_lds_bytes<Cfg>() <= 160 * 1024 &&
                  (kWsmTH * kTW * Cfg::COUT_TILE * 2) % (16 * kThreads * 2) == 0) {
        if (a.pss && a.n_chunks == 1 && a.n_ct == 4 && a.cin_vec_ok && a.cin_chunk_ok && a.persist_ok && n_tiles < (1 << 24)) {
            if (report(0, legacy_slots)) return RC_OK;
            constexpr int PSS_LDS = pss_lds_bytes<Cfg>();
            const int n_items = a.tiles_x * ((a.H + kWsmTH - 1) / kWsmTH) * a.batch;
            return launch_lds<&conv_mfma_pss_kernel<Cfg>>(dim3((unsigned)persistent_grid(a.num_cus, n_items)), dim3(kWsmThreads), PSS_LDS, stream, a);
        }
    }
    constexpr int WSM_LDS = wsm_lds_bytes<Cfg>();
    if constexpr (!GATED && WSM_LDS <= 160 * 1024 && Cfg::KS >= 2 && Cfg::STEPS >= 2 && sizeof(typename Cfg::elem) == 2) {
        const bool res_pre_form = FAST && !GATED && sizeof(typename Cfg::elem) == 2 && Cfg::NT <= 3 && a.ep_key == ConvDev<Cfg>::EP_RES && a.out_mode == RC_OUT_NHWC;
        if ((a.n_chunks > 1 || (a.n_ct > 1 && a.persist_ok != 3 && !(P_OK && res_pre_form))) && a.cin_vec_ok && a.cin_chunk_ok && a.persist_ok && a.cout_packed <= kPersistMaxCout &&
            n_tiles < (1 << 24)) {
            if (report(0, legacy_slots)) return RC_OK;
            { int c_; if (int e_ = sums_mode(0, c_)) return e_; }
            const int n_items = a.tiles_x * ((a.H + kWsmTH - 1) / kWsmTH) * a.batch * (a.n_chunks > 1 ? a.n_ct : 1);
            const int grid = persistent_grid(a.num_cus, n_items);
            if constexpr ((FAST || Cfg::NT <= 3) && wst_eligible<Cfg>()) {
                if (a.thin >= (wst_form<Cfg>() == 3 ? 1 : 2)) return launch_wst<Cfg, FAST>(a, grid, stream);
            }
            return launch_lds<&conv_mfma_wsm_kernel<Cfg, GATED, FAST>>(dim3((unsigned)grid), dim3(kWsmThreads), WSM_LDS, stream, a);
        }
    }
    if constexpr (!GATED && FAST && auto64_eligible<Cfg>()) {
        using DD = ConvDev<Cfg>;
        const int k7 = a.ep_key;
        const bool key_ok = k7 == 0 || k7 == DD::EP_RELU || k7 == DD::EP_LEAKY || k7 == DD::EP_SUMS || k7 == (DD::EP_RELU | DD::EP_SUMS) || k7 == (DD::EP_LEAKY | DD::EP_SUMS) ||
                            k7 == DD::EP_RES || (k7 == (DD::EP_GATE | DD::EP_RES) && a.batch * a.cout <= kAutoGate);
        if (a.auto_impl && key_ok && a.n_chunks == 1 && a.n_ct == 1 && a.cout == Cfg::COUT_TILE && a.cin_vec_ok && a.persist_ok && a.out_mode == RC_OUT_NHWC && n_tiles < (1 << 24)) {
            constexpr int A_LDS = auto64_lds_bytes<Cfg>();
            static_assert(A_LDS <= 160 * 1024, "kernel 7 LDS");
            const int grid = persistent_grid(a.num_cus, (n_tiles + 1) / 2);
            const int cslots = ((k7 & DD::EP_SUMS) && a.sums_compact_ok && grid * 8 < legacy_slots) ? grid * 8 : 0;
            if (report(7, cslots ? cslots : legacy_slots)) return RC_OK;
            ConvArgs aa = a;
            if (int e_ = sums_mode(cslots, aa.sums_compact)) return e_;
            if (k7 & DD::EP_SUMS) return launch_lds<&conv_mfma_auto64_kernel<Cfg, 1>>(dim3((unsigned)grid), dim3(kAutoThreads), A_LDS, stream, aa);
            if (k7 & DD::EP_RES) return launch_lds<&conv_mfma_auto64_kernel<Cfg, 2>>(dim3((unsigned)grid), dim3(kAutoThreads), A_LDS, stream, aa);
            return launch_lds<&conv_mfma_auto64_kernel<Cfg, 0>>(dim3((unsigned)grid), dim3(kAutoThreads), A_LDS, stream, aa);
        }
    }
    if constexpr (!GATED && FAST && auto_eligible<Cfg>()) {
        using DD = ConvDev<Cfg>;
        const bool key_ok = a.ep_key >= 0 && (a.ep_key & (DD::EP_FILM | DD::EP_MUL)) == 0 && (a.ep_key != (DD::EP_GATE | DD::EP_RES) || a.batch * a.cout <= kAutoGate);
        const bool mode_ok = a.auto_impl == 2 || (a.ep_key & DD::EP_RES) == 0;
        if (a.auto_impl && key_ok && mode_ok && a.n_chunks == 1 && a.n_ct == 1 && a.cin_vec_ok && a.persist_ok && a.out_mode == RC_OUT_NHWC && n_tiles < (1 << 24)) {
            constexpr int A_LDS = auto_lds_bytes<Cfg>();
            const int n_items = a.tiles_x * ((a.H + kWsmTH - 1) / kWsmTH) * a.batch;
            const int grid = persistent_grid(a.num_cus, n_items);
            const bool run_sums = a.ep_key == DD::EP_SUMS || a.ep_key == (DD::EP_RELU | DD::EP_SUMS);
            const int cslots = (run_sums && a.sums_compact_ok && grid * 8 < legacy_slots) ? grid * 8 : 0;
            if (report(6, cslots ? cslots : legacy_slots)) return RC_OK;
            ConvArgs aa = a;
            if (int e_ = sums_mode(cslots, aa.sums_compact)) return e_;
            if (run_sums) return launch_lds<&conv_mfma_auto_kernel<Cfg, 1>>(dim3((unsigned)grid), dim3(kAutoThreads), A_LDS, stream, aa);
            if (a.ep_key == DD::EP_RES || a.ep_key == (DD::EP_GATE | DD::EP_RES))
                return launch_lds<&conv_mfma_auto_kernel<Cfg, 2>>(dim3((unsigned)grid), dim3(kAutoThreads), A_LDS, stream, aa);
            return launch_lds<&conv_mfma_auto_kernel<Cfg, 0>>(dim3((unsigned)grid), dim3(kAutoThreads), A_LDS, stream, aa);
        }
    }
    if constexpr (P_OK && !GATED) {
        if (a.n_chunks == 1 && a.cout_packed <= persist_bias_slots<Cfg>() && a.persist_ok && n_tiles < (1 << 24)) {
            const bool one_per_cu = (a.dbg_flags & 64) != 0 && P_LDS <= 80 * 1024;
            const int grid = persistent_grid((one_per_cu ? 1 : persist_blocks_per_cu<Cfg>()) * a.num_cus, n_tiles);
            const bool run_sums = FAST && sizeof(typename Cfg::elem) == 2 && Cfg::NT >= 3 && a.n_ct == 1 &&
                                  (a.ep_key == ConvDev<Cfg>::EP_SUMS || a.ep_key == (ConvDev<Cfg>::EP_RELU | ConvDev<Cfg>::EP_SUMS));
            const int cslots = (run_sums && a.sums_compact_ok && grid * 4 < legacy_slots) ? grid * 4 : 0;
            if (report(2, cslots ? cslots : legacy_slots)) return RC_OK;
            ConvArgs aa = a;
            if (int e_ = sums_mode(cslots, aa.sums_compact)) return e_;
            const int lds_res = P_LDS + (a.n_ct - 1) * (int)Cfg::CHUNK_W_BYTES;
            aa.w_resident = (a.n_ct > 1 && lds_res <= 80 * 1024 && !(a.dbg_flags & 128)) ? 1 : 0;
            const int lds_bytes = one_per_cu ? 100 * 1024 : (aa.w_resident ? lds_res : P_LDS);
// ... 21 lines not shown
```

### realcamnet_amd/networks.py

```python
from __future__ import annotations

from collections import OrderedDict

import torch
import torch.nn as nn

from . import ops
from ._lib import RC_OUT_NHWC, RC_OUT_PIXEL_SHUFFLE2


def _is_act(m) -> bool:
    return isinstance(m, (nn.ReLU, nn.LeakyReLU)) or (isinstance(m, nn.GELU) and m.approximate == "none")


def _act_args(m):
    if isinstance(m, nn.ReLU):
        return dict(act="relu")
    if isinstance(m, nn.GELU):
        return dict(act="gelu")
    return dict(act="leaky", slope=float(m.negative_slope))


class HipModule(nn.Module):

    def forward(self, x):
        a = ops.to_nhwc(x)
        return ops.to_nchw(self._nhwc(a))

    def _nhwc(self, a):
        raise NotImplementedError


class Conv2d(nn.Conv2d):

    def forward(self, x):
        return ops.to_nchw(self._nhwc(ops.to_nhwc(x)))

    def _nhwc(self, a, **fuse):
        if ops.is_down2x2(self):
            return ops.conv2x2s2(a, self, **fuse)
        if tuple(self.stride) == (2, 2) and ops.is_stride2(self):
            return ops.conv_stride2(a, self, **fuse)
        return ops.conv2d(a, self, **fuse)


class Sequential(nn.Sequential):

    def forward(self, x):
        if isinstance(x, (tuple, list)):
            a = (ops.to_nhwc(x[0]), *x[1:])
            y = self._nhwc(a)
            return (ops.to_nchw(y[0]), *y[1:])
        return ops.to_nchw(self._nhwc(ops.to_nhwc(x)))

    def _nhwc(self, a, residual=None):
        mods = list(self)
        i, n = 0, len(mods)
        while i < n:
            m = mods[i]
            if isinstance(m, Conv2d):
                kw = {}
                j = i + 1
                if j < n and _is_act(mods[j]):
                    kw.update(_act_args(mods[j]))
                    j += 1
                shuffle_after = False
                if j < n and isinstance(mods[j], nn.PixelShuffle):
                    if mods[j].upscale_factor != 2:
                        raise NotImplementedError("PixelShuffle: only upscale_factor=2 is on the hot path")
                    if (m.out_channels // 4) % 16 == 0:
                        kw["out_mode"] = RC_OUT_PIXEL_SHUFFLE2
                    else:
                        shuffle_after = True
                    j += 1
                if (j < n and isinstance(mods[j], DWTForward) and "out_mode" not in kw and not shuffle_after and
                        ops.conv_dwt_ok(a, m, mods[j], kw.get("act"), kw.get("slope", 0.0))):
                    kw["out_mode"] = ops.RC_OUT_NHWC_DWT
                    j += 1
                if j == n and residual is not None and kw.get("out_mode", RC_OUT_NHWC) == RC_OUT_NHWC and not shuffle_after:
                    kw["residual"], residual = residual, None
                a = m._nhwc(a, **kw)
                if shuffle_after:
                    a = ops.pixel_shuffle2(a)
                i = j
                continue
            if isinstance(m, RCAGroup) and i + 1 < n and isinstance(mods[i + 1], DWTForward) and not isinstance(a, (tuple, list)):
                a = m._nhwc(a, dwt=mods[i + 1])
                i += 2
                continue
            if isinstance(m, (nn.Dropout, nn.Identity)):
                i += 1
                continue
            if not hasattr(m, "_nhwc"):
                raise NotImplementedError(f"{type(m).__name__} has no HIP implementation on this path")
            a = m._nhwc(a)
            i += 1
        if residual is not None:
            raise NotImplementedError("trailing residual could not be fused (sequence does not end in a conv)")
        return a


def seq(*args):
    if len(args) == 1:
        args = args[0]
    if isinstance(args, nn.Module):
        return args
    if isinstance(args, OrderedDict):
        return Sequential(OrderedDict((k, seq(v)) for k, v in args.items()))
    assert isinstance(args, (list, tuple))
    return Sequential(*[seq(i) for i in args])


_UNSUPPORTED = "XTBIiSP34UuMA"


def conv(in_channels=64, out_channels=64, kernel_size=3, stride=1, padding=1, output_padding=0, dilation=1,
         groups=1, bias=True, padding_mode='zeros', mode='CBR'):
    L = []
    for t in mode:
        if t == 'C':
            L.append(Conv2d(in_channels=in_channels, out_channels=out_channels, kernel_size=kernel_size,
                            stride=stride, padding=padding, dilation=dilation, groups=groups, bias=bias,
                            padding_mode=padding_mode))
        elif t == 'R':
            L.append(nn.ReLU(inplace=True))
        elif t == 'r':
            L.append(nn.ReLU(inplace=False))
        elif t == 'L':
            L.append(nn.LeakyReLU(negative_slope=1e-1, inplace=True))
        elif t == 'l':
            L.append(nn.LeakyReLU(negative_slope=1e-1, inplace=False))
        elif t == '2':
            L.append(nn.PixelShuffle(upscale_factor=2))
        elif t in _UNSUPPORTED:
            raise NotImplementedError(f"conv mode '{t}' is not on the RAW->sRGB hot path (SURVEY.md section 8); no HIP kernel")
        else:
            raise NotImplementedError('Undefined type: {}'.format(t))
    return seq(*L)


_HAAR = [[[[0.5, 0.5], [0.5, 0.5]]],
         [[[0.5, 0.5], [-0.5, -0.5]]],
         [[[0.5, -0.5], [0.5, -0.5]]],
         [[[0.5, -0.5], [-0.5, 0.5]]]]


class DWTForward(nn.Conv2d):

    def __init__(self, in_channels=64):
        super().__init__(in_channels, in_channels * 4, 2, 2, groups=in_channels, bias=False)
        w = torch.tensor(_HAAR, dtype=torch.get_default_dtype()).repeat(in_channels, 1, 1, 1)
        self.weight.data.copy_(w)
        self.requires_grad_(False)

    def forward(self, x):
        return ops.to_nchw(self._nhwc(ops.to_nhwc(x)))

    def _nhwc(self, a):
        return ops.dwt_forward(a, self)


class DWTInverse(nn.ConvTranspose2d):

    def __init__(self, in_channels=64):
        super().__init__(in_channels, in_channels // 4, 2, 2, groups=in_channels // 4, bias=False)
        w = torch.tensor(_HAAR, dtype=torch.get_default_dtype()).repeat(in_channels // 4, 1, 1, 1)
        self.weight.data.copy_(w)
        self.requires_grad_(False)

    def forward(self, x, output_size=None):
        return ops.to_nchw(self._nhwc(ops.to_nhwc(x)))

    def _nhwc(self, a):
        return ops.dwt_inverse(a, self)


class DWTForward_(nn.Module):

    def __init__(self):
        super().__init__()
        ll, lh, hl, hh = [[0.5, 0.5], [0.5, 0.5]], [[-0.5, -0.5], [0.5, 0.5]], [[-0.5, 0.5], [-0.5, 0.5]], [[0.5, -0.5], [-0.5, 0.5]]
# ... 141 lines not shown
```

### realcamnet_amd/ops.py

```python
from __future__ import annotations

import ctypes as C
import math
from typing import Optional, Tuple

import numpy as np
import os
import torch
from torch._subclasses.fake_tensor import FakeTensor

from . import _lib
from . import torch_ops as _T
from ._lib import (RC_ACT_GELU, RC_ACT_LEAKY, RC_ACT_NONE, RC_ACT_RELU, RC_ACT_RELU_POST, RC_BF16, RC_F16, RC_F32, RC_OUT_NCHW, RC_OUT_NHWC, RC_OUT_NHWC_DWT,
                   RC_OUT_PIXEL_SHUFFLE2, RC_OUT_PIXEL_SHUFFLE2_NCHW, ConvDesc, ConvPairDesc, check)

_DT = {torch.float32: RC_F32, torch.bfloat16: RC_BF16, torch.float16: RC_F16}
_HALF = (torch.bfloat16, torch.float16)
_R = torch.ops.realcam


def _opt(t: torch.Tensor) -> Optional[torch.Tensor]:
    return t if t.numel() else None

FUSE_GATE = True


def lib():
    return _lib.load()


def _dt(t: torch.Tensor) -> int:
    try:
        return _DT[t.dtype]
    except KeyError:
        raise TypeError(f"realcamnet_amd: unsupported dtype {t.dtype} (fp32 / bf16 / fp16)") from None


def require_dtype(t: torch.Tensor, allowed, what: str) -> None:
    if t.dtype not in allowed:
        names = " / ".join({torch.float32: "fp32", torch.bfloat16: "bf16", torch.float16: "fp16"}.get(d, str(d)) for d in allowed)
        raise TypeError(f"realcamnet_amd: {what} supports {names} only, got {t.dtype}")


def _req(t: torch.Tensor, name: str) -> torch.Tensor:
    if not isinstance(t, torch.Tensor):
        raise TypeError(f"{name}: expected a tensor")
    if not t.is_cuda:
        raise RuntimeError(f"{name}: tensor is on {t.device}; the HIP path has no CPU fallback "
                           "(use oracle/ for CPU reference results)")
    return t if t.is_contiguous() else t.contiguous()


def _stream() -> int:
    return torch.cuda.current_stream().cuda_stream


def _ptr(t: Optional[torch.Tensor]) -> Optional[int]:
    return None if t is None else t.data_ptr()


def derived(mod, slot, params, build, extra=None):
    cache = mod.__dict__.get("_rc_cache")
    if cache is None:
        cache = mod.__dict__["_rc_cache"] = {}
    key = (tuple(None if p is None else (id(p), 0 if isinstance(p, FakeTensor) else p.data_ptr(), p._version, p.dtype, str(p.device)) for p in params), extra)
    hit = cache.get(slot)
    if hit is not None and hit[0] == key:
        return hit[2]
    cache.pop(slot, None)
    value = build()
    cache[slot] = (key, tuple(params), value)
    return value


def drop_derived(mod, *slots) -> None:
    if not slots:
        mod.__dict__.pop("_rc_cache", None)
    for slot in slots:
        mod.__dict__.get("_rc_cache", {}).pop(slot, None)


def invalidate_caches(module) -> None:
    for m in module.modules():
        for k in ("_rc_cache", "_f32_masters", "_f32_verdict", "_graphs"):
            m.__dict__.pop(k, None)


def f32_param(mod, name: str) -> torch.Tensor:
    p = getattr(mod, name)
    if p.dtype == torch.float32 and p.is_contiguous():
        return _req(p.detach(), name)
    return derived(mod, ("f32", name), (p,), lambda: _req(p.detach(), name).float().contiguous())


class PackedConv:
    __slots__ = ("wpacked", "bias", "cin", "cout", "ksize", "dtype", "out_mode")
# ... 725 lines not shown
    roi = stats.check(h, w)
    hist, zones = _R.frame_stats(y, h, w, list(roi), stats.grid[0], stats.grid[1], stats.bits, MATRICES[stats.matrix], stats.dark_code, stats.clip_code)
    return FrameStats(hist, zones, stats, roi)


def make_coord(b: int, h: int, w: int, device=None, dtype: torch.dtype = torch.float32) -> torch.Tensor:
    ys = torch.linspace(-1.0, 1.0, h, device=device).view(1, 1, h, 1).expand(b, 1, h, w)
    xs = torch.linspace(-1.0, 1.0, w, device=device).view(1, 1, 1, w).expand(b, 1, h, w)
    return torch.cat([ys, xs], dim=1).to(dtype).contiguous()


_ACT = {None: RC_ACT_NONE, "relu": RC_ACT_RELU, "leaky": RC_ACT_LEAKY, "gelu": RC_ACT_GELU, "relu_post": RC_ACT_RELU_POST}


SMALL_MAP_COUT_TILE = os.environ.get("RC_SMALL_MAP_COUT_TILE", "1") != "0"
_CU_COUNT = {}
_SMALL_MAP_FACTOR = int(os.environ.get("RC_SMALL_MAP_FACTOR", "2"))


def small_map_cout_tile(x: torch.Tensor, mod, out_mode: int) -> int:
    w = mod.weight
    if not SMALL_MAP_COUT_TILE or x.dtype != torch.float32 or w.dim() != 4 or w.shape[-1] != 3 or w.shape[0] % 64 != 0 or w.shape[1] % 16 != 0:
        return 0
    if out_mode not in (RC_OUT_NHWC, RC_OUT_NCHW):
        return 0
    dev = x.device.index if x.device.index is not None else 0
    cus = _CU_COUNT.get(dev)
    if cus is None:
        try:
            cus = torch.cuda.get_device_properties(dev).multi_processor_count if x.is_cuda else 256
        except (RuntimeError, AssertionError):
            cus = 256
        _CU_COUNT[dev] = cus
    b, H, W, _ = x.shape
    blocks = b * ((H + 7) // 8) * ((W + 31) // 32) * (w.shape[0] // 64)
    return 16 if blocks < _SMALL_MAP_FACTOR * cus else 0


WINOGRAD = os.environ.get("RC_WINOGRAD", "1") != "0"


def winograd_ok(x: torch.Tensor, mod, *, act=None, gate=None, skip=None, mul_plus1=None, out_mode: int = RC_OUT_NHWC, store_input: bool = False) -> bool:
    w = mod.weight
    if not WINOGRAD or x.dtype != torch.float32 or w.dim() != 4 or tuple(w.shape[2:]) != (3, 3):
        return False
    if w.shape[1] % 8 != 0 or w.shape[0] % 64 != 0 or out_mode != RC_OUT_NHWC:
        return False
    if gate is not None or skip is not None or mul_plus1 is not None or store_input or act == "gelu":
        return False
    return True


def packed_wino(mod, act_dtype: torch.dtype) -> PackedConv:
    w, b = mod.weight, mod.bias

    def pack():
        if not w.is_cuda:
            raise RuntimeError("conv weights are not on a HIP device; move the module with .cuda() first")
        pc = PackedConv()
        pc.wpacked = _R.wino_pack_weights(w.detach(), act_dtype)
        pc.bias = b.detach().float().contiguous() if b is not None else None
        pc.cout, pc.cin, pc.ksize, pc.dtype, pc.out_mode = w.shape[0], w.shape[1], 3, _DT[act_dtype], RC_OUT_NHWC
        return pc
    return derived(mod, ("wino", act_dtype), (w, b), pack)


def conv2d(x: torch.Tensor, mod, *, act: Optional[str] = None, slope: float = 0.0,
           residual: Optional[torch.Tensor] = None, mul_plus1: Optional[torch.Tensor] = None,
           film: Optional[Tuple[torch.Tensor, torch.Tensor]] = None,
           gate: Optional[torch.Tensor] = None, skip: Optional[torch.Tensor] = None, store_input: bool = False,
           out_mode: int = RC_OUT_NHWC, want_sums: bool = False,
           crop_hw: Optional[Tuple[int, int]] = None, out_dtype: Optional[torch.dtype] = None,
           out_scale: Optional[torch.Tensor] = None):
    if mod.weight.dim() == 4:
        check_conv_module(mod)
    x = _req(x, "conv input")
    b, H, W, cin = x.shape
    algo = 1 if mod.weight.dim() == 4 and winograd_ok(x, mod, act=act, gate=gate, skip=skip, mul_plus1=mul_plus1, out_mode=out_mode, store_input=store_input) else 0
    if algo:
        ct = 0
        pc = packed_wino(mod, x.dtype)
    else:
        ct = small_map_cout_tile(x, mod, out_mode)
        pc = packed_conv(mod, x.dtype, RC_OUT_NHWC if out_mode == RC_OUT_NHWC_DWT else out_mode, ct)
    if cin != pc.cin:
        raise ValueError(f"conv expects {pc.cin} input channels, got {cin}")
    if gate is not None:
        if skip is None:
            raise ValueError("gate needs skip")
        skip = _req(skip, "skip")
        gate = _req(gate, "gate")
        if skip.shape != x.shape or skip.dtype != x.dtype or gate.shape != (b, cin) or gate.dtype != torch.float32:
            raise ValueError("gate/skip shape or dtype mismatch")
    fs = ft = None
    if film is not None:
        fs, ft = (_req(t, "film") for t in film)
        if fs.shape != (b, pc.cout) or ft.shape != (b, pc.cout) or fs.dtype != torch.float32 or ft.dtype != torch.float32:
            raise ValueError("film tensors must be fp32 (B, cout)")
    if mul_plus1 is not None:
        mul_plus1 = _req(mul_plus1, "mul_plus1")
    if out_scale is not None:
        out_scale = _req(out_scale, "out_scale")
        if out_scale.shape != (b, pc.cout) or out_scale.dtype != torch.float32 or out_mode != RC_OUT_NHWC:
            raise ValueError("out_scale must be fp32 (B, cout) and needs the NHWC store")
    if residual is not None:
        residual = _req(residual, "residual")
    for name, t in (("mul_plus1", mul_plus1), ("residual", residual)):
        if t is not None and (t.shape != (b, H, W, pc.cout) or t.dtype != x.dtype):
            raise ValueError(f"{name} must be NHWC {(b, H, W, pc.cout)} {x.dtype}, got {tuple(t.shape)} {t.dtype}")
    planar = out_mode in (RC_OUT_NCHW, RC_OUT_PIXEL_SHUFFLE2_NCHW)
    ch, cw = (crop_hw if crop_hw is not None else (0, 0)) if planar else (0, 0)
    if out_dtype is not None:
        _DT[out_dtype]
    out, stored, sums = _R.conv2d(x, pc.wpacked, pc.bias, pc.cout, pc.ksize, _ACT[act], float(slope), residual, mul_plus1, fs, ft, gate, skip,
                                  bool(store_input), int(out_mode), bool(want_sums), int(ch), int(cw),
                                  out_dtype if planar else None, out_scale, ct, algo)
    extras = [t for t in (_opt(stored), _opt(sums)) if t is not None]
    return (out, *extras) if extras else out


FUSE_DWT = os.environ.get("RC_FUSE_DWT", "1") != "0"
_HAAR_TAPS = (0.5, 0.5, 0.5, 0.5, 0.5, 0.5, -0.5, -0.5, 0.5, -0.5, 0.5, -0.5, 0.5, -0.5, -0.5, 0.5)


def conv_dwt_ok(x: torch.Tensor, conv, dwt, act: Optional[str] = None, slope: float = 0.0, residual: bool = False) -> bool:
    if residual and act is not None:
        return False
    if not FUSE_DWT or x.dtype not in _HALF or x.dim() != 4 or conv.weight.dim() != 4:
        return False
    cout, cin, kh, kw = conv.weight.shape
    if not (kh == kw == 3 and cin == cout and cin in (32, 48) and x.shape[3] == cin and x.shape[1] % 2 == 0 and x.shape[2] % 2 == 0):
        return False
    if tuple(conv.stride) != (1, 1) or tuple(conv.padding) != (1, 1) or tuple(conv.dilation) != (1, 1) or conv.groups != 1:
        return False
    if act not in (None, "relu", "leaky") or (act == "leaky" and not (0.0 <= slope <= 1.0)):
        return False
    w = getattr(dwt, "weight", None)
    if w is None or tuple(w.shape) != (4 * cout, 1, 2, 2):
        return False
    if isinstance(w, FakeTensor):
        return True

    def taps_are_haar():
        want = torch.tensor(_HAAR_TAPS, dtype=torch.float32).reshape(4, 1, 2, 2).repeat(cout, 1, 1, 1)
        return bool(torch.equal(w.detach().float().cpu(), want))
    return derived(dwt, "haar_ok", (w,), taps_are_haar)


FUSE_SHUFFLE_STORE = True

FOLD_TAIL = True


def tail_fold_ok(x: torch.Tensor, conv1, conv2) -> bool:
    w1, w2 = conv1.weight, conv2.weight
    if not (FOLD_TAIL and x.dim() == 4 and x.dtype in _DT and x.shape[1] >= 2 and x.shape[2] >= 2 and w1.dim() == 4 and w2.dim() == 4):
        return False
    c = x.shape[-1]
    return (tuple(w1.shape) == (4 * c, c, 3, 3) and tuple(w2.shape[1:]) == (c, 3, 3) and 4 * w2.shape[0] <= 16 and
            _lib.load().rc_conv_packed_bytes(c, 4 * w2.shape[0], 5, _DT[x.dtype], RC_OUT_PIXEL_SHUFFLE2_NCHW) != 0)


def _folded_tail(conv1, conv2) -> "_ConvView":
    def fold():
        det = lambda t: None if t is None else t.detach()
        wc, bc = _R.tail_fold_weights(conv1.weight.detach(), det(conv1.bias), conv2.weight.detach(), det(conv2.bias))
        c = conv1.weight.shape[1]
        perm = (torch.arange(c, device=conv1.weight.device)[:, None] * 4 + torch.tensor([0, 2, 1, 3], device=conv1.weight.device)[None, :]).reshape(-1)
        v1t = _ConvView(conv1.weight.detach().transpose(2, 3)[perm].contiguous(), None if conv1.bias is None else conv1.bias.detach()[perm].contiguous())
        v2t = _ConvView(conv2.weight.detach().transpose(2, 3).contiguous(), det(conv2.bias))
        return _ConvView(wc, bc), v1t, v2t
    return derived(conv2, "tail_fold", (conv1.weight, conv1.bias, conv2.weight, conv2.bias), fold)


def tail_fold(x: torch.Tensor, conv1, conv2, crop_hw: Optional[Tuple[int, int]] = None, out_dtype: Optional[torch.dtype] = None) -> torch.Tensor:
    x = _req(x, "tail input")
    b, H, W, _ = x.shape
    odt = out_dtype or x.dtype

    folded, c1t, c2t = _folded_tail(conv1, conv2)

    def ring():
        rows, cols_t = _R.tail_ring_gather(x)
        return [conv2d(conv2d(t, m1, out_mode=RC_OUT_PIXEL_SHUFFLE2), m2, out_mode=RC_OUT_NCHW, out_dtype=odt) for t, m1, m2 in ((rows, conv1, conv2), (cols_t, c1t, c2t))]

    strips, out = fork_join(ring, lambda: conv2d(x, folded, out_mode=RC_OUT_PIXEL_SHUFFLE2_NCHW, crop_hw=crop_hw, out_dtype=odt), [x])
    _R.tail_ring_scatter(out, strips[0], strips[1], H, W)
    return out


FUSE_PAIR = False


def conv_pair_ok(x: torch.Tensor, m1, m2) -> bool:
    return (FUSE_PAIR and x.dtype == torch.bfloat16 and x.shape[-1] == 48 and
            all(m.weight.dim() == 4 and tuple(m.weight.shape) == (48, 48, 3, 3) for m in (m1, m2)))


def conv_pair(x: torch.Tensor, m1, m2, *, act: str = "relu", slope: float = 0.0,
              film: Optional[Tuple[torch.Tensor, torch.Tensor]] = None,
              gate: Optional[torch.Tensor] = None, skip: Optional[torch.Tensor] = None, store_input: bool = False,
              residual: Optional[torch.Tensor] = None, want_sums: bool = False):
    require_dtype(x, (torch.bfloat16,), "conv_pair (rc_conv_pair)")
    for m in (m1, m2):
        check_conv_module(m)
    x = _req(x, "conv_pair input")
    b, H, W, c = x.shape
    p1, p2 = packed_conv(m1, x.dtype, RC_OUT_NHWC), packed_conv(m2, x.dtype, RC_OUT_NHWC)
    if gate is not None:
        if skip is None:
            raise ValueError("gate needs skip")
        skip, gate = _req(skip, "skip"), _req(gate, "gate")
        if skip.shape != x.shape or skip.dtype != x.dtype or gate.shape != (b, c) or gate.dtype != torch.float32:
            raise ValueError("gate/skip shape or dtype mismatch")
    fs = ft = None
    if film is not None:
        fs, ft = (_req(t, "film") for t in film)
        if fs.shape != (b, c) or ft.shape != (b, c) or fs.dtype != torch.float32 or ft.dtype != torch.float32:
            raise ValueError("film tensors must be fp32 (B, C)")
    if residual is not None:
        residual = _req(residual, "residual")
        if residual.shape != x.shape or residual.dtype != x.dtype:
            raise ValueError("residual must match the input tensor")
    out, stored, sums = _R.conv_pair(x, p1.wpacked, p1.bias, p2.wpacked, p2.bias, _ACT[act], float(slope), fs, ft, gate, skip, bool(store_input),
                                     residual, bool(want_sums))
    extras = [t for t in (_opt(stored), _opt(sums)) if t is not None]
    return (out, *extras) if extras else out


FUSE_CHAIN = True

# ... 362 lines not shown
```

### realcamnet_amd/torch_ops.py

```python
from __future__ import annotations

import ctypes as C
from typing import List, Optional

import numpy as np
import torch
from torch import Tensor

from . import _lib
from ._lib import RC_BF16, RC_F16, RC_F32, RC_OUT_NCHW, RC_OUT_NHWC, RC_OUT_NHWC_DWT, RC_OUT_PIXEL_SHUFFLE2, RC_OUT_PIXEL_SHUFFLE2_NCHW, ConvDesc, ConvPairDesc, check

_DT = {torch.float32: RC_F32, torch.bfloat16: RC_BF16, torch.float16: RC_F16}
_LIB = torch.library.Library("realcam", "DEF")
SCHEMAS = {}


def lib():
    return _lib.load()


def _dt(t: Tensor) -> int:
    return _DT[t.dtype]


def _stream() -> int:
    return torch.cuda.current_stream().cuda_stream


def _p(t: Optional[Tensor]):
    return None if t is None else t.data_ptr()


def _none(x: Tensor) -> Tensor:
    return x.new_empty((0,))


def require_acts(op: str, dtype, *tensors) -> None:
    for t in tensors:
        if t is None:
            continue
        if t.dtype != dtype:
            raise TypeError(f"realcam::{op}: activation tensor of dtype {t.dtype}, expected {dtype}")
        if not t.is_contiguous():
            raise ValueError(f"realcam::{op}: non-contiguous activation tensor (shape {tuple(t.shape)}, strides {t.stride()})")


def define(schema: str, alloc, launch, acts=None):
    name = schema.split("(")[0]
    SCHEMAS[name] = schema
    _LIB.define(schema)

    def cuda_impl(*args):
        if acts is not None:
            require_acts(name, *acts(*args))
        outs = alloc(*args)
        launch(outs, *args)
        return outs

    def fake_impl(*args):
        return alloc(*args)

    _LIB.impl(name, cuda_impl, "CUDA")
    torch.library.register_fake(f"realcam::{name}", fake_impl, lib=_LIB)


def _bu_alloc(mosaic, dtype, pad_to):
    b, h2, w2 = mosaic.shape
    h, w = h2 // 2, w2 // 2
    return mosaic.new_empty((b, -(-h // pad_to) * pad_to, -(-w // pad_to) * pad_to, 4), dtype=dtype)


def _bu_launch(out, mosaic, dtype, pad_to):
    b, h2, w2 = mosaic.shape
    check(lib().rc_bayer_unshuffle(mosaic.data_ptr(), _dt(mosaic), out.data_ptr(), _DT[dtype], b, h2 // 2, w2 // 2, out.shape[1], out.shape[2],
                                   _stream()), "rc_bayer_unshuffle")


define("bayer_unshuffle(Tensor mosaic, ScalarType dtype, int pad_to) -> Tensor", _bu_alloc, _bu_launch)


def _ingest_alloc(mosaic, dtype, pad_to, black, white, cond_h, cond_w):
    b, h2, w2 = mosaic.shape
    h, w = h2 // 2, w2 // 2
    return (mosaic.new_empty((b, -(-h // pad_to) * pad_to, -(-w // pad_to) * pad_to, 4), dtype=dtype),
            mosaic.new_empty((b, 4, cond_h, cond_w), dtype=dtype))


def _ingest_launch(outs, mosaic, dtype, pad_to, black, white, cond_h, cond_w):
    packed, cond = outs
    b, h2, w2 = mosaic.shape
    in_dt = _lib.RC_U16 if mosaic.dtype == torch.uint16 else _dt(mosaic)
    check(lib().rc_raw_ingest(mosaic.data_ptr(), in_dt, packed.data_ptr(), cond.data_ptr(), _DT[dtype], b, h2 // 2, w2 // 2,
                              packed.shape[1], packed.shape[2], cond_h, cond_w, float(black), float(white), _stream()), "rc_raw_ingest")
# ... 288 lines not shown


def _quad_launch(out, src, storage, cfa, width, mode):
    b, h, _ = src.shape
    src, f = _raw_source(src, storage, cfa, width, (0.0,) * 4, 0.0)
    d = _lib.QuadDesc(mode=mode)
    check(lib().rc_raw_quad(src.data_ptr(), C.byref(f), C.byref(d), out.data_ptr(), 0, b, h, width, _stream()), "rc_raw_quad")


define("raw_quad(Tensor src, int storage, int cfa, int width, int mode) -> Tensor", _quad_alloc, _quad_launch)

define("nchw_to_nhwc(Tensor x, ScalarType dtype, int hp, int wp) -> Tensor",
       lambda x, dtype, hp, wp: x.new_empty((x.shape[0], hp, wp, x.shape[1]), dtype=dtype),
       lambda out, x, dtype, hp, wp: check(lib().rc_nchw_to_nhwc(x.data_ptr(), _dt(x), out.data_ptr(), _DT[dtype], x.shape[0], x.shape[1],
                                                                 x.shape[2], x.shape[3], hp, wp, _stream()), "rc_nchw_to_nhwc"))

define("nhwc_to_nchw(Tensor a, ScalarType dtype, int h, int w) -> Tensor",
       lambda a, dtype, h, w: a.new_empty((a.shape[0], a.shape[3], h, w), dtype=dtype),
       lambda out, a, dtype, h, w: check(lib().rc_nhwc_to_nchw(a.data_ptr(), _dt(a), out.data_ptr(), _DT[dtype], a.shape[0], a.shape[3],
                                                               a.shape[1], a.shape[2], h, w, _stream()), "rc_nhwc_to_nchw"))


def _wshape(weight):
    if weight.dim() == 2:
        return weight.shape[0], weight.shape[1], 1
    return weight.shape[0], weight.shape[1], weight.shape[2]


def _pack_alloc(weight, bias, act_dtype, out_mode, cout_tile=0):
    cout, cin, k = _wshape(weight)
    L = lib()
    dt = _DT[act_dtype]
    nbytes = L.rc_conv_packed_bytes_ct(cin, cout, k, dt, out_mode, cout_tile)
    if nbytes == 0:
        raise _lib.HipError(f"rc_conv_packed_bytes: {L.rc_last_error().decode()}")
    n_packed = L.rc_conv_packed_cout_ct(cin, cout, k, dt, out_mode, cout_tile)
    return (weight.new_empty((nbytes,), dtype=torch.uint8),
            weight.new_empty((n_packed if bias is not None else 0,), dtype=torch.float32))


def _pack_launch(outs, weight, bias, act_dtype, out_mode, cout_tile=0):
    wp, bp = outs
    cout, cin, k = _wshape(weight)
    L = lib()
    dt = _DT[act_dtype]
    w_host = np.ascontiguousarray(weight.detach().float().cpu().numpy())
    dst = np.empty(wp.numel(), dtype=np.uint8)
    check(L.rc_conv_pack_weights_ct(w_host.ctypes.data, cin, cout, k, dt, out_mode, cout_tile, dst.ctypes.data), "rc_conv_pack_weights")
    wp.copy_(torch.from_numpy(dst))
    if bias is not None:
        b_host = np.ascontiguousarray(bias.detach().float().cpu().numpy())
        bdst = np.zeros(bp.numel(), dtype=np.float32)
        check(L.rc_conv_pack_bias_ct(b_host.ctypes.data, cin, cout, k, dt, out_mode, cout_tile, bdst.ctypes.data), "rc_conv_pack_bias")
        bp.copy_(torch.from_numpy(bdst))


define("conv_pack_weights(Tensor weight, Tensor? bias, ScalarType act_dtype, int out_mode, int cout_tile=0) -> (Tensor, Tensor)", _pack_alloc, _pack_launch)


def _wino_pack_alloc(weight, act_dtype):
    cout, cin, k = _wshape(weight)
    nbytes = lib().rc_wino_packed_bytes(cin, cout, _DT[act_dtype]) if k == 3 else 0
    if nbytes == 0:
        raise _lib.HipError(f"rc_wino_packed_bytes: {lib().rc_last_error().decode() if k == 3 else 'a 3x3 form'}")
    return weight.new_empty((nbytes,), dtype=torch.uint8)


def _wino_pack_launch(out, weight, act_dtype):
    cout, cin, _ = _wshape(weight)
    w_host = np.ascontiguousarray(weight.detach().float().cpu().numpy())
    dst = np.empty(out.numel(), dtype=np.uint8)
    check(lib().rc_wino_pack_weights(w_host.ctypes.data, cin, cout, _DT[act_dtype], dst.ctypes.data), "rc_wino_pack_weights")
    out.copy_(torch.from_numpy(dst))


define("wino_pack_weights(Tensor weight, ScalarType act_dtype) -> Tensor", _wino_pack_alloc, _wino_pack_launch)


def _conv_alloc(x, wpacked, bias, cout, ksize, act, slope, residual, mul_plus1, film_scale, film_shift, gate, skip, store_input, out_mode,
                want_sums, crop_h, crop_w, out_dtype, out_scale=None, cout_tile=0, algo=0):
    b, H, W, _ = x.shape
    if out_mode == RC_OUT_NHWC:
        out = x.new_empty((b, H, W, cout))
    elif out_mode == RC_OUT_PIXEL_SHUFFLE2:
        out = x.new_empty((b, 2 * H, 2 * W, cout // 4))
    elif out_mode == RC_OUT_NHWC_DWT:
        out = x.new_empty((b, H // 2, W // 2, 4 * cout))
    elif out_mode == RC_OUT_PIXEL_SHUFFLE2_NCHW:
        out = x.new_empty((b, cout // 4, crop_h if crop_h > 0 else 2 * H, crop_w if crop_w > 0 else 2 * W), dtype=out_dtype or x.dtype)
    else:
        out = x.new_empty((b, cout, crop_h if crop_h > 0 else H, crop_w if crop_w > 0 else W), dtype=out_dtype or x.dtype)
    stored = torch.empty_like(x) if (store_input and gate is not None) else _none(x)
    sums = x.new_empty((0,), dtype=torch.float32)
    if want_sums:
        d = ConvDesc()
        d.batch, d.height, d.width, d.cin, d.cout, d.ksize, d.dtype = b, H, W, x.shape[-1], cout, ksize, _DT[x.dtype]
        from torch._subclasses.fake_tensor import FakeTensor

        def stand_in(t):
            return 4096 + (0 if (t is None or isinstance(t, FakeTensor) or not t.is_cuda) else t.data_ptr() % 16)
        d.in0, d.wpacked, d.out, d.chan_sums = stand_in(x), stand_in(wpacked), stand_in(out), 4096
        if gate is not None:
            d.in1, d.in_gate = stand_in(skip), stand_in(gate)
            if store_input:
                d.in_store = 4096
        for name, t in (("bias", bias), ("film_scale", film_scale), ("film_shift", film_shift), ("mul_plus1", mul_plus1), ("residual", residual), ("out_scale", out_scale)):
            if t is not None:
                setattr(d, name, stand_in(t))
        d.act, d.act_slope, d.out_mode, d.out_dtype = act, float(slope), out_mode, _DT[out.dtype]
        d.cout_tile = cout_tile
        d.algo = algo
        if out_mode in (RC_OUT_NCHW, RC_OUT_PIXEL_SHUFFLE2_NCHW):
            d.out_h, d.out_w = out.shape[2], out.shape[3]
        if x.is_cuda and not isinstance(x, FakeTensor):
            with torch.cuda.device(x.device):
                n = lib().rc_conv_sum_slots(C.byref(d))
        else:
            n = lib().rc_conv_sum_slots(C.byref(d))
        if n <= 0:
            n = lib().rc_conv_sum_tiles(H, W)
        sums = x.new_empty((b, n, cout), dtype=torch.float32)
    return out, stored, sums


def _conv_launch(outs, x, wpacked, bias, cout, ksize, act, slope, residual, mul_plus1, film_scale, film_shift, gate, skip, store_input,
                 out_mode, want_sums, crop_h, crop_w, out_dtype, out_scale=None, cout_tile=0, algo=0):
    out, stored, sums = outs
    b, H, W, cin = x.shape
    d = ConvDesc()
    d.batch, d.height, d.width, d.cin, d.cout, d.ksize, d.dtype = b, H, W, cin, cout, ksize, _dt(x)
    d.in0 = x.data_ptr()
    if gate is not None:
        d.in1, d.in_gate = skip.data_ptr(), gate.data_ptr()
        if stored.numel():
            d.in_store = stored.data_ptr()
    d.wpacked, d.bias = wpacked.data_ptr(), _p(bias)
    d.film_scale, d.film_shift = _p(film_scale), _p(film_shift)
    d.act, d.act_slope = act, float(slope)
    d.mul_plus1, d.residual, d.out_scale = _p(mul_plus1), _p(residual), _p(out_scale)
    d.out, d.out_mode = out.data_ptr(), out_mode
    d.out_dtype = _dt(out)
    d.cout_tile = cout_tile
    d.algo = algo
    if out_mode in (RC_OUT_NCHW, RC_OUT_PIXEL_SHUFFLE2_NCHW):
        d.out_h, d.out_w = out.shape[2], out.shape[3]
    if want_sums:
        d.chan_sums = sums.data_ptr()
        d.chan_sums_slots = sums.shape[1]
    check(lib().rc_conv2d(C.byref(d), _stream()), "rc_conv2d")


define("conv2d(Tensor x, Tensor wpacked, Tensor? bias, int cout, int ksize, int act, float slope, Tensor? residual, Tensor? mul_plus1, "
       "Tensor? film_scale, Tensor? film_shift, Tensor? gate, Tensor? skip, bool store_input, int out_mode, bool want_sums, "
       "int crop_h, int crop_w, ScalarType? out_dtype, Tensor? out_scale=None, int cout_tile=0, int algo=0) -> (Tensor, Tensor, Tensor)", _conv_alloc, _conv_launch)


def _conv_fold2_launch(out, x, wpacked, bias, cout, act, slope):
    b, H, W, c = x.shape
    d = ConvDesc()
    d.batch, d.height, d.width, d.cin, d.cout, d.ksize, d.dtype = b, (H + 1) // 2, (W + 1) // 2, 4 * c, cout, 2, _dt(x)
    d.src_h, d.src_w = H, W
    d.in0, d.wpacked, d.bias = x.data_ptr(), wpacked.data_ptr(), _p(bias)
    d.act, d.act_slope = act, float(slope)
    d.out, d.out_mode, d.out_dtype = out.data_ptr(), RC_OUT_NHWC, _dt(out)
    check(lib().rc_conv2d(C.byref(d), _stream()), "rc_conv2d")


# ... 590 lines not shown
```

Before: 1331 MP/s.

## Fuse inverse Haar DWT into preceding 3x3 conv epilogue for decoder stages

Adds an RC_OUT_NHWC_IDWT output mode in which the last conv of the middle and up blocks applies the inverse Haar wavelet in its epilogue. The result is written directly at 2x resolution with cout/4 channels, and the next up block skips its leading DWTInverse. This removes a separate IDWT kernel and a full write plus re-read of the low-resolution tensor for each of three decoder levels. In exchange it adds lane-permute shuffles and restricts the path to bf16 3x3 layers with specific cin/cout shapes, with a fallback to the unfused path otherwise.

```diff
diff --git a/include/realcam_hip.h b/include/realcam_hip.h
--- a/include/realcam_hip.h
+++ b/include/realcam_hip.h
@@ -29,7 +29,8 @@
     RC_OUT_PIXEL_SHUFFLE2 = 1,
     RC_OUT_NCHW = 2,
     RC_OUT_PIXEL_SHUFFLE2_NCHW = 3,
-    RC_OUT_NHWC_DWT = 4
+    RC_OUT_NHWC_DWT = 4,
+    RC_OUT_NHWC_IDWT = 5
 } rc_out_mode;
 
 int rc_abi_version(void);
diff --git a/realcamnet_amd/LiteISP.py b/realcamnet_amd/LiteISP.py
--- a/realcamnet_amd/LiteISP.py
+++ b/realcamnet_amd/LiteISP.py
@@ -452,10 +452,16 @@
         d1 = self._refine_d1(self.down1._nhwc(h))
         d2 = self.down2._nhwc(mod(2, d1))
         d3 = self.down3._nhwc(mod(3, d2))
-        m = self.middle._nhwc(mod(4, d3), residual=d3)
-        u3 = self.up3._nhwc(m, residual=d2)
-        u2 = self.up2._nhwc(u3, residual=d1)
-        u1 = self.up1._nhwc(u2, residual=h)
+        if ops.FUSE_IDWT and all(isinstance(u[0], N.DWTInverse) for u in (self.up3, self.up2, self.up1)):
+            m = self.middle._nhwc(mod(4, d3), residual=d3, idwt=self.up3[0])
+            u3 = self.up3._nhwc(m, residual=d2, idwt=self.up2[0], skip_first=True)
+            u2 = self.up2._nhwc(u3, residual=d1, idwt=self.up1[0], skip_first=True)
+            u1 = self.up1._nhwc(u2, residual=h, skip_first=True)
+        else:
+            m = self.middle._nhwc(mod(4, d3), residual=d3)
+            u3 = self.up3._nhwc(m, residual=d2)
+            u2 = self.up2._nhwc(u3, residual=d1)
+            u1 = self.up1._nhwc(u2, residual=h)
         if ops.tail_fold_ok(u1, self.tail[0], self.tail[2]):
             return ops.tail_fold(u1, self.tail[0], self.tail[2], crop_hw=crop_hw, out_dtype=self.output_dtype)
         t = self.tail[0]._nhwc(u1, out_mode=RC_OUT_PIXEL_SHUFFLE2)
diff --git a/realcamnet_amd/_lib.py b/realcamnet_amd/_lib.py
--- a/realcamnet_amd/_lib.py
+++ b/realcamnet_amd/_lib.py
@@ -11,7 +11,7 @@
 
 RC_F32, RC_BF16, RC_U16, RC_F16 = 0, 1, 2, 3
 RC_ACT_NONE, RC_ACT_RELU, RC_ACT_LEAKY, RC_ACT_GELU, RC_ACT_RELU_POST = 0, 1, 2, 3, 4
-RC_OUT_NHWC, RC_OUT_PIXEL_SHUFFLE2, RC_OUT_NCHW, RC_OUT_PIXEL_SHUFFLE2_NCHW, RC_OUT_NHWC_DWT = 0, 1, 2, 3, 4
+RC_OUT_NHWC, RC_OUT_PIXEL_SHUFFLE2, RC_OUT_NCHW, RC_OUT_PIXEL_SHUFFLE2_NCHW, RC_OUT_NHWC_DWT, RC_OUT_NHWC_IDWT = 0, 1, 2, 3, 4, 5
 ABI_VERSION = 15
 RC_RAW_F32, RC_RAW_BF16, RC_RAW_U16, RC_RAW_F16, RC_RAW_U8, RC_RAW_MIPI10, RC_RAW_MIPI12 = 0, 1, 2, 3, 4, 5, 6
 RC_CFA_RGGB, RC_CFA_BGGR, RC_CFA_GRBG, RC_CFA_GBRG = 0, 1, 2, 3
diff --git a/realcamnet_amd/csrc/conv.hip b/realcamnet_amd/csrc/conv.hip
--- a/realcamnet_amd/csrc/conv.hip
+++ b/realcamnet_amd/csrc/conv.hip
@@ -341,11 +341,19 @@
 static int conv_build_args(const rc_conv_desc* d, ConvPlan& p, ConvArgs& a, size_t& es_out) {
     RC_REQUIRE(d != nullptr, "rc_conv2d: null desc");
     const bool dwt = d->out_mode == RC_OUT_NHWC_DWT;
-    RC_REQUIRE(make_plan(d->cin, d->cout, d->ksize, d->dtype, dwt ? (int)RC_OUT_NHWC : d->out_mode, &p, d->cout_tile), "rc_conv2d: unsupported cin/cout/ksize/dtype/cout_tile");
+    const bool idwt = d->out_mode == RC_OUT_NHWC_IDWT;
+    RC_REQUIRE(make_plan(d->cin, d->cout, d->ksize, d->dtype, (dwt || idwt) ? (int)RC_OUT_NHWC : d->out_mode, &p, d->cout_tile), "rc_conv2d: unsupported cin/cout/ksize/dtype/cout_tile");
     RC_REQUIRE(d->batch >= 1 && d->height >= 1 && d->width >= 1, "rc_conv2d: empty tensor");
     RC_REQUIRE(d->batch <= 65535, "rc_conv2d: batch > 65535");
     RC_REQUIRE(d->in0 && d->wpacked && d->out, "rc_conv2d: null in0/wpacked/out");
-    RC_REQUIRE(d->out_mode >= RC_OUT_NHWC && d->out_mode <= RC_OUT_NHWC_DWT, "rc_conv2d: bad out_mode");
+    RC_REQUIRE(d->out_mode >= RC_OUT_NHWC && d->out_mode <= RC_OUT_NHWC_IDWT, "rc_conv2d: bad out_mode");
+    if (idwt) {
+        RC_REQUIRE(d->out_dtype == d->dtype && reinterpret_cast<uintptr_t>(d->out) % 16 == 0, "rc_conv2d: RC_OUT_NHWC_IDWT: out_dtype must equal dtype, out 16-byte aligned");
+        RC_REQUIRE(!d->mul_plus1 && !d->film_scale && !d->out_scale && !d->chan_sums && !d->in_gate && !d->in1 && !d->in_store && !d->src_h && !d->src_w && !d->cout_tile,
+                   "rc_conv2d: RC_OUT_NHWC_IDWT excludes mul_plus1 / film / out_scale / chan_sums / gated input / src_h / cout_tile");
+        if (d->dtype != RC_BF16 || d->ksize != 3 || p.m32 || d->act != RC_ACT_NONE || d->cout % 4 != 0 || d->cout != p.cout_packed)
+            return fail(RC_ERR_UNSUPPORTED, "rc_conv2d: RC_OUT_NHWC_IDWT is a bf16 3x3 form with act NONE, cout % 4 == 0 and whole cout tiles");
+    }
     if (dwt) {
         RC_REQUIRE(d->height % 2 == 0 && d->width % 2 == 0, "rc_conv2d: RC_OUT_NHWC_DWT needs even height and width");
         RC_REQUIRE(d->out_dtype == d->dtype && reinterpret_cast<uintptr_t>(d->out) % 16 == 0, "rc_conv2d: RC_OUT_NHWC_DWT: out_dtype must equal dtype, out 16-byte aligned");
@@ -361,7 +369,7 @@
     RC_REQUIRE((d->film_scale == nullptr) == (d->film_shift == nullptr), "rc_conv2d: film_scale/film_shift must come together");
     const bool full_tiles = d->cout == p.cout_packed;
     if (d->mul_plus1 || d->residual)
-        RC_REQUIRE((full_tiles || d->cout % 4 == 0) && (d->out_mode == RC_OUT_NHWC || (dwt && !d->mul_plus1)), "rc_conv2d: mul_plus1/residual need cout % 4 == 0 and RC_OUT_NHWC (residual: or RC_OUT_NHWC_DWT)");
+        RC_REQUIRE((full_tiles || d->cout % 4 == 0) && (d->out_mode == RC_OUT_NHWC || ((dwt || idwt) && !d->mul_plus1)), "rc_conv2d: mul_plus1/residual need cout % 4 == 0 and RC_OUT_NHWC (residual: or RC_OUT_NHWC_DWT / RC_OUT_NHWC_IDWT)");
     if (d->chan_sums) RC_REQUIRE(d->out_mode == RC_OUT_NHWC, "rc_conv2d: chan_sums needs RC_OUT_NHWC");
     if (d->out_scale) {
         RC_REQUIRE(d->out_mode == RC_OUT_NHWC && !p.m32, "rc_conv2d: out_scale needs RC_OUT_NHWC and a layer outside the 32x32x16 forms");
@@ -369,7 +377,7 @@
     }
     const size_t es = dtype_size(d->dtype);
     const int planar16 = d->dtype == RC_F16 ? RC_F16 : RC_BF16;
-    if (dwt) {
+    if (dwt || idwt) {
     } else if (d->out_mode == RC_OUT_NHWC) {
         RC_REQUIRE(d->out_dtype == d->dtype, "rc_conv2d: out_dtype must equal dtype for RC_OUT_NHWC");
         RC_REQUIRE(!full_tiles || (d->cout * es) % 8 == 0, "rc_conv2d: cout*elem_size must be a multiple of 8 bytes for RC_OUT_NHWC");
diff --git a/realcamnet_amd/csrc/conv_kernel.hpp b/realcamnet_amd/csrc/conv_kernel.hpp
--- a/realcamnet_amd/csrc/conv_kernel.hpp
+++ b/realcamnet_amd/csrc/conv_kernel.hpp
@@ -928,6 +928,103 @@
             __builtin_amdgcn_raw_buffer_store_b128(u32x4_t{o[4 * i], o[4 * i + 1], o[4 * i + 2], o[4 * i + 3]}, r_out, oo, 16 * i, 0);
     }
 
+    __device__ static __forceinline__ void rows_transpose4(unsigned (&r)[4]) {
+        u32x2_t s;
+        s = __builtin_amdgcn_permlane32_swap(r[0], r[2], false, false); r[0] = s.x; r[2] = s.y;
+        s = __builtin_amdgcn_permlane32_swap(r[1], r[3], false, false); r[1] = s.x; r[3] = s.y;
+        s = __builtin_amdgcn_permlane16_swap(r[0], r[1], false, false); r[0] = s.x; r[1] = s.y;
+        s = __builtin_amdgcn_permlane16_swap(r[2], r[3], false, false); r[2] = s.x; r[3] = s.y;
+    }
+    template <bool PRE>
+    __device__ static __forceinline__ void epilogue_idwt(const ConvArgs& a, int b, int y0, int x0, int ct, int tid, f32x4 (&acc)[4][NT],
+                                                         const unsigned (&rp)[PRE ? 4 : 1][PRE ? NV / 2 : 1]) {
+        static_assert(ES == 2 && (NV == 12 || NV == 16), "16-bit storage; 48- or 64-wide cout tiles");
+        typedef float f32x2 __attribute__((ext_vector_type(2)));
+        constexpr int NC = NV / 4;
+        const int lane = tid & 63, wave = tid >> 6, q = lane >> 4, n = lane & 15;
+        const int jbase = ct * Cfg::COUT_TILE + q * NV;
+        const size_t img_out = (size_t)a.H * a.W * a.cout;
+        const unsigned img_bytes = (unsigned)(img_out * ES);
+        const __amdgpu_buffer_rsrc_t r_out = make_rsrc(static_cast<T*>(a.out) + (size_t)b * img_out, img_bytes);
+        const int gy = y0 + 2 * wave, gx = x0 + n;
+        const int row_b = a.W * a.cout * ES, col_b = 16 * a.cout * ES;
+        const int off0 = ((gy * a.W + gx) * a.cout + jbase) * ES;
+        const int cps = a.cout >> 2;
+        const int o_pix = cps * ES, o_line = 2 * a.W * cps * ES;
+        const int o_off0 = (((2 * gy + (q >> 1)) * (2 * a.W) + 2 * gx + (q & 1)) * cps + ct * (Cfg::COUT_TILE / 4)) * ES;
+        [[maybe_unused]] const int o_dir0 = ((2 * gy * (2 * a.W) + 2 * gx) * cps + (jbase >> 2)) * ES;
+        const bool has_res = a.residual != nullptr;
+#pragma unroll
+        for (int pt = 0; pt < 4; ++pt) {
+            const int dy = pt >> 1, dx = pt & 1;
+            const bool valid = gy + dy < a.H && gx + 16 * dx < a.W;
+            float v[NV];
+#pragma unroll
+            for (int nt = 0; nt < NT; ++nt)
+#pragma unroll
+                for (int r = 0; r < 4; ++r) v[nt * 4 + r] = acc[pt][nt][r];
+            if (has_res) {
+                if constexpr (PRE) {
+#pragma unroll
+                    for (int i = 0; i < NV / 2; ++i) {
+                        v[2 * i] += lo16<T>(rp[pt][i]);
+                        v[2 * i + 1] += hi16<T>(rp[pt][i]);
+                    }
+                } else {
+                    float m[NV];
+                    buf_load_row<T, NV>(make_rsrc(static_cast<const T*>(a.residual) + (size_t)b * img_out, img_bytes), valid ? off0 + dy * row_b + dx * col_b : kOOB, m);
+#pragma unroll
+                    for (int e = 0; e < NV; ++e) v[e] += m[e];
+                }
+            }
+            float h[NV];
+#pragma unroll
+            for (int i = 0; i < NV / 2; ++i) {
+                const unsigned w = pack16x2<T>(v[2 * i], v[2 * i + 1]);
+                h[2 * i] = lo16<T>(w);
+                h[2 * i + 1] = hi16<T>(w);
+            }
+            float o[4][NC];
+#pragma unroll
+            for (int c = 0; c + 1 < NC; c += 2) {
+                const f32x2 k0 = f32x2{h[4 * c], h[4 * c + 4]} * 0.5f, k1 = f32x2{h[4 * c + 1], h[4 * c + 5]} * 0.5f;
+                const f32x2 k2 = f32x2{h[4 * c + 2], h[4 * c + 6]} * 0.5f, k3 = f32x2{h[4 * c + 3], h[4 * c + 7]} * 0.5f;
+                const f32x2 sab = k0 + k1, dab = k0 - k1;
+                const f32x2 o0 = (sab + k2) + k3, o1 = (sab - k2) - k3, o2 = (dab + k2) - k3, o3 = (dab - k2) + k3;
+                o[0][c] = o0.x; o[0][c + 1] = o0.y; o[1][c] = o1.x; o[1][c + 1] = o1.y;
+                o[2][c] = o2.x; o[2][c + 1] = o2.y; o[3][c] = o3.x; o[3][c + 1] = o3.y;
+            }
+            if constexpr (NC % 2 != 0) {
+                constexpr int c = NC - 1;
+                const float k0 = h[4 * c] * 0.5f, k1 = h[4 * c + 1] * 0.5f, k2 = h[4 * c + 2] * 0.5f, k3 = h[4 * c + 3] * 0.5f;
+                const float sab = k0 + k1, dab = k0 - k1;
+                o[0][c] = (sab + k2) + k3;
+                o[1][c] = (sab - k2) - k3;
+                o[2][c] = (dab + k2) - k3;
+                o[3][c] = (dab - k2) + k3;
+            }
+            unsigned wa[4], wb[4];
+#pragma unroll
+            for (int t = 0; t < 4; ++t) {
+                wa[t] = pack16x2<T>(o[t][0], o[t][1]);
+                wb[t] = pack16x2<T>(o[t][2], NC == 4 ? o[t][NC - 1] : 0.f);
+            }
+            if constexpr (NC == 4) {
+                const int od = (valid && !(a.dbg_flags & 1)) ? o_dir0 + dy * 2 * o_line + dx * 32 * o_pix : kOOB;
+#pragma unroll
+                for (int t = 0; t < 4; ++t) __builtin_amdgcn_raw_buffer_store_b64(u32x2_t{wa[t], wb[t]}, r_out, od, (t >> 1) * o_line + (t & 1) * o_pix, 0);
+            } else {
+                rows_transpose4(wa);
+                rows_transpose4(wb);
+                const int oo = (valid && !(a.dbg_flags & 1)) ? o_off0 + dy * 2 * o_line + dx * 32 * o_pix : kOOB;
+                const unsigned d1 = __builtin_amdgcn_perm(wa[1], wb[0], 0x05040100u), d2 = __builtin_amdgcn_perm(wb[1], wa[1], 0x05040302u);
+                const unsigned d4 = __builtin_amdgcn_perm(wa[3], wb[2], 0x05040100u), d5 = __builtin_amdgcn_perm(wb[3], wa[3], 0x05040302u);
+                __builtin_amdgcn_raw_buffer_store_b128(u32x4_t{wa[0], d1, d2, wa[2]}, r_out, oo, 0, 0);
+                __builtin_amdgcn_raw_buffer_store_b64(u32x2_t{d4, d5}, r_out, oo + 16, 0, 0);
+            }
+        }
+    }
+
     __device__ static __forceinline__ void epilogue_generic(const ConvArgs& a, int b, int y0, int x0, int sp, int ct, int tid,
                                                             f32x4 (&acc)[4][NT]) {
         const int lane = tid & 63, wave = tid >> 6, q = lane >> 4, n = lane & 15;
@@ -1152,7 +1249,7 @@
 template <class Cfg>
 constexpr int persist_blocks_per_cu() { return Cfg::NT <= 2 && persist_lds_bytes_c<Cfg>() * 3 <= 160 * 1024 ? 3 : 2; }
 
-template <class Cfg, bool GATED, bool FAST>
+template <class Cfg, bool GATED, bool FAST, bool IDWT = false>
 __global__ __launch_bounds__(kThreads, persist_blocks_per_cu<Cfg>()) void conv_mfma_persist_kernel(const ConvArgs a) {
     using D = ConvDev<Cfg>;
     constexpr int NT = Cfg::NT, STEPS = Cfg::STEPS, NV = 4 * NT;
@@ -1251,15 +1348,18 @@
             }
             constexpr bool RESPRE = FAST && !GATED && sizeof(typename Cfg::elem) == 2 && NT <= 3;
             [[maybe_unused]] unsigned rpre[RESPRE ? 4 : 1][RESPRE ? D::NRH : 1];
-            bool res_pre = false;
+            [[maybe_unused]] bool res_pre = false;
             if constexpr (RESPRE) {
-                if ((a.ep_key == D::EP_RES || a.ep_key == (D::EP_GATE | D::EP_RES)) && a.out_mode == RC_OUT_NHWC) {
+                if (IDWT ? a.residual != nullptr : ((a.ep_key == D::EP_RES || a.ep_key == (D::EP_GATE | D::EP_RES)) && a.out_mode == RC_OUT_NHWC)) {
                     res_pre = true;
                     D::res_prefetch(a, cb, cy0, cx0, ct, tid, rpre);
                 }
             }
             D::template mma_steps<0, STEPS, 0, (!GATED && NT < 5)>(s_in, a.w_resident ? s_w + ct * (int)Cfg::CHUNK_W_BYTES : s_w, lane_x, lane_w, q, lo, acc);
-            if constexpr (FAST && sizeof(typename Cfg::elem) == 2) {
+            if constexpr (IDWT) {
+                static_assert(RESPRE, "the IDWT form prefetches its residual");
+                D::template epilogue_idwt<true>(a, cb, cy0, cx0, ct, tid, acc, rpre);
+            } else if constexpr (FAST && sizeof(typename Cfg::elem) == 2) {
                 const int rslot = a.sums_compact ? 4 * D::compact_residue(pos, cb, sp_total, (int)gridDim.x) : -1;
                 if (RUN_SUMS && a.ep_key == D::EP_SUMS && n_ct == 1)
                     D::template epilogue_fast_impl<D::EP_SUMS, RUN_SUMS>(a, cb, cy0, cx0, csp, ct, tid, acc, run, tile < 0 || b != cb, rslot);
@@ -1554,7 +1654,7 @@
 constexpr bool wst_eligible() { return wst_form<Cfg>() != 0; }
 constexpr int waitcnt_vm(int n) { return (n & 15) | ((n >> 4) << 14) | 0x0F70; }
 
-template <class Cfg8, bool FAST>
+template <class Cfg8, bool FAST, bool IDWT = false>
 __global__ __launch_bounds__(kWsmThreads) void conv_mfma_wst_kernel(const ConvArgs a) {
 #if defined(__HIP_DEVICE_COMPILE__)
     using Cfg = WstCfg<Cfg8>;
@@ -1757,8 +1857,12 @@
                 } else {
                     run_chunks(std::integral_constant<int, 3>{}, 0, n_chunks);
                 }
-                if (ty8 < a.tiles_y)
-                    D8::template epilogue<FAST>(a, b, ty8 * kTH, tx * kTW, ty8 * a.tiles_x + tx, ct, tid & 255, acc);
+                if (ty8 < a.tiles_y) {
+                    if constexpr (IDWT) {
+                        const unsigned nor[1][1] = {{0u}};
+                        D8::template epilogue_idwt<false>(a, b, ty8 * kTH, tx * kTW, ct, tid & 255, acc, nor);
+                    } else D8::template epilogue<FAST>(a, b, ty8 * kTH, tx * kTW, ty8 * a.tiles_x + tx, ct, tid & 255, acc);
+                }
                 __syncthreads();
             }
             kb3 = kb3 == NBUF - 1 ? 0 : kb3 + 1;
@@ -2310,6 +2414,14 @@
 template <class Cfg, bool FAST>
 int launch_wst(const ConvArgs& a, int grid, hipStream_t stream) {
     return launch_lds<&conv_mfma_wst_kernel<Cfg, FAST>>(dim3((unsigned)grid), dim3(kWsmThreads), wst_lds_bytes<Cfg>(), stream, a);
+}
+
+template <class Cfg>
+constexpr int idwt_form() {
+    if (!(dtype_of<typename Cfg::elem>::value == RC_BF16 && Cfg::KS == 3)) return 0;
+    if (Cfg::CK == 48 && Cfg::NT == 3 && persist_lds_bytes_c<Cfg>() <= 80 * 1024) return 2;
+    if (Cfg::CK == 32 && Cfg::NT == 4 && wst_form<Cfg>() == 2) return 4;
+    return 0;
 }
 
 template <class Cfg, bool GATED, bool FAST>
@@ -2345,6 +2457,28 @@
         }
         return fail(RC_ERR_UNSUPPORTED, "rc_conv2d: RC_OUT_NHWC_DWT needs a bf16 / fp16 3x3 layer of one Cin chunk and one 32- or 48-wide cout tile (cin == cout == 32 or 48), 16-byte aligned operands");
     }
+    if (a.out_mode == RC_OUT_NHWC_IDWT) {
+        if constexpr (!GATED && FAST && idwt_form<Cfg>() != 0) {
+            using DD = ConvDev<Cfg>;
+            if ((a.ep_key == 0 || a.ep_key == DD::EP_RES) && (idwt_form<Cfg>() == 2 ? a.n_chunks == 1 : a.n_chunks > 1) && a.cin_vec_ok && a.cin_chunk_ok &&
+                a.cout == a.cout_packed && a.cout_packed <= kPersistMaxCout && n_tiles < (1 << 24)) {
+                if (report(0, legacy_slots)) return RC_OK;
+                if constexpr (idwt_form<Cfg>() == 2) {
+                    const int grid = persistent_grid(persist_blocks_per_cu<Cfg>() * a.num_cus, n_tiles);
+                    ConvArgs aa = a;
+                    const int lds_res = P_LDS + (a.n_ct - 1) * (int)Cfg::CHUNK_W_BYTES;
+                    aa.w_resident = (a.n_ct > 1 && lds_res <= 80 * 1024) ? 1 : 0;
+                    if (int e_ = allow_lds<&conv_mfma_persist_kernel<Cfg, false, true, true>>(P_LDS > 100 * 1024 ? P_LDS : 100 * 1024)) return e_;
+                    return launch_lds<&conv_mfma_persist_kernel<Cfg, false, true, true>>(dim3((unsigned)grid), dim3(kThreads), aa.w_resident ? lds_res : P_LDS, stream, aa);
+                } else {
+                    const int n_items = a.tiles_x * ((a.H + kWsmTH - 1) / kWsmTH) * a.batch * a.n_ct;
+                    return launch_lds<&conv_mfma_wst_kernel<Cfg, true, true>>(dim3((unsigned)persistent_grid(a.num_cus, n_items)), dim3(kWsmThreads), wst_lds_bytes<Cfg>(), stream, a);
+                }
+            }
+        }
+        return fail(RC_ERR_UNSUPPORTED, "rc_conv2d: RC_OUT_NHWC_IDWT needs a bf16 3x3 layer with cout % 4 == 0 of one 48-channel Cin chunk and 48-wide cout tiles (cin == 48, cout % 48 == 0) or of "
+                                        "several 32-channel chunks and 64-wide cout tiles (cin % 64 == 0, cin > 64, cout % 64 == 0), cout <= 512, 16-byte aligned operands");
+    }
     constexpr int WS_LDS = ws_lds_bytes<Cfg>();
     if constexpr (WS_LDS <= 150 * 1024) {
         const bool ws_auto = GATED || Cfg::NT == 5 || Cfg::CK == 80;
diff --git a/realcamnet_amd/networks.py b/realcamnet_amd/networks.py
--- a/realcamnet_amd/networks.py
+++ b/realcamnet_amd/networks.py
@@ -53,9 +53,13 @@
             return (ops.to_nchw(y[0]), *y[1:])
         return ops.to_nchw(self._nhwc(ops.to_nhwc(x)))
 
-    def _nhwc(self, a, residual=None):
+    def _nhwc(self, a, residual=None, idwt=None, skip_first=False):
         mods = list(self)
         i, n = 0, len(mods)
+        if skip_first:
+            if not (n and isinstance(mods[0], DWTInverse)):
+                raise NotImplementedError("skip_first: the sequence does not open with a DWTInverse")
+            i = 1
         while i < n:
             m = mods[i]
             if isinstance(m, Conv2d):
@@ -79,6 +83,9 @@
                     j += 1
                 if j == n and residual is not None and kw.get("out_mode", RC_OUT_NHWC) == RC_OUT_NHWC and not shuffle_after:
                     kw["residual"], residual = residual, None
+                if (j == n and idwt is not None and residual is None and kw.get("out_mode", RC_OUT_NHWC) == RC_OUT_NHWC and not shuffle_after and "act" not in kw and
+                        ops.conv_idwt_ok(a, m, idwt, kw.get("residual"))):
+                    kw["out_mode"], idwt = ops.RC_OUT_NHWC_IDWT, None
                 a = m._nhwc(a, **kw)
                 if shuffle_after:
                     a = ops.pixel_shuffle2(a)
@@ -97,6 +104,8 @@
             i += 1
         if residual is not None:
             raise NotImplementedError("trailing residual could not be fused (sequence does not end in a conv)")
+        if idwt is not None:
+            a = idwt._nhwc(a)
         return a
 
 
diff --git a/realcamnet_amd/ops.py b/realcamnet_amd/ops.py
--- a/realcamnet_amd/ops.py
+++ b/realcamnet_amd/ops.py
@@ -11,7 +11,7 @@
 
 from . import _lib
 from . import torch_ops as _T
-from ._lib import (RC_ACT_GELU, RC_ACT_LEAKY, RC_ACT_NONE, RC_ACT_RELU, RC_ACT_RELU_POST, RC_BF16, RC_F16, RC_F32, RC_OUT_NCHW, RC_OUT_NHWC, RC_OUT_NHWC_DWT,
+from ._lib import (RC_ACT_GELU, RC_ACT_LEAKY, RC_ACT_NONE, RC_ACT_RELU, RC_ACT_RELU_POST, RC_BF16, RC_F16, RC_F32, RC_OUT_NCHW, RC_OUT_NHWC, RC_OUT_NHWC_DWT, RC_OUT_NHWC_IDWT,
                    RC_OUT_PIXEL_SHUFFLE2, RC_OUT_PIXEL_SHUFFLE2_NCHW, ConvDesc, ConvPairDesc, check)
 
 _DT = {torch.float32: RC_F32, torch.bfloat16: RC_BF16, torch.float16: RC_F16}
@@ -903,7 +903,7 @@
         pc = packed_wino(mod, x.dtype)
     else:
         ct = small_map_cout_tile(x, mod, out_mode)
-        pc = packed_conv(mod, x.dtype, RC_OUT_NHWC if out_mode == RC_OUT_NHWC_DWT else out_mode, ct)
+        pc = packed_conv(mod, x.dtype, RC_OUT_NHWC if out_mode in (RC_OUT_NHWC_DWT, RC_OUT_NHWC_IDWT) else out_mode, ct)
     if cin != pc.cin:
         raise ValueError(f"conv expects {pc.cin} input channels, got {cin}")
     if gate is not None:
@@ -968,6 +968,42 @@
     return derived(dwt, "haar_ok", (w,), taps_are_haar)
 
 
+FUSE_IDWT = os.environ.get("RC_FUSE_IDWT", "1") != "0"
+IDWT_FORMS = frozenset(("k2", "k4b"))
+
+
+def conv_idwt_form(cin: int, cout: int) -> Optional[str]:
+    if cout % 4 or cout > 512:
+        return None
+    if cin == 48 and cout % 48 == 0:
+        return "k2"
+    if cin % 64 == 0 and cin > 64 and cout % 64 == 0:
+        return "k4b"
+    return None
+
+
+def conv_idwt_ok(x: torch.Tensor, conv, idwt, residual: Optional[torch.Tensor] = None) -> bool:
+    if not FUSE_IDWT or x.dtype != torch.bfloat16 or x.dim() != 4 or conv.weight.dim() != 4:
+        return False
+    cout, cin, kh, kw = conv.weight.shape
+    if not (kh == kw == 3 and x.shape[3] == cin and conv_idwt_form(cin, cout) in IDWT_FORMS):
+        return False
+    if tuple(conv.stride) != (1, 1) or tuple(conv.padding) != (1, 1) or tuple(conv.dilation) != (1, 1) or conv.groups != 1:
+        return False
+    if residual is not None and (tuple(residual.shape) != (*x.shape[:3], cout) or residual.dtype != x.dtype):
+        return False
+    w = getattr(idwt, "weight", None)
+    if w is None or tuple(w.shape) != (cout, 1, 2, 2) or tuple(getattr(idwt, "stride", ())) != (2, 2):
+        return False
+    if isinstance(w, FakeTensor):
+        return True
+
+    def taps_are_haar():
+        want = torch.tensor(_HAAR_TAPS, dtype=torch.float32).reshape(4, 1, 2, 2).repeat(cout // 4, 1, 1, 1)
+        return bool(torch.equal(w.detach().float().cpu(), want))
+    return derived(idwt, "haar_ok", (w,), taps_are_haar)
+
+
 FUSE_SHUFFLE_STORE = True
 
 FOLD_TAIL = True
diff --git a/realcamnet_amd/torch_ops.py b/realcamnet_amd/torch_ops.py
--- a/realcamnet_amd/torch_ops.py
+++ b/realcamnet_amd/torch_ops.py
@@ -8,7 +8,7 @@
 from torch import Tensor
 
 from . import _lib
-from ._lib import RC_BF16, RC_F16, RC_F32, RC_OUT_NCHW, RC_OUT_NHWC, RC_OUT_NHWC_DWT, RC_OUT_PIXEL_SHUFFLE2, RC_OUT_PIXEL_SHUFFLE2_NCHW, ConvDesc, ConvPairDesc, check
+from ._lib import RC_BF16, RC_F16, RC_F32, RC_OUT_NCHW, RC_OUT_NHWC, RC_OUT_NHWC_DWT, RC_OUT_NHWC_IDWT, RC_OUT_PIXEL_SHUFFLE2, RC_OUT_PIXEL_SHUFFLE2_NCHW, ConvDesc, ConvPairDesc, check
 
 _DT = {torch.float32: RC_F32, torch.bfloat16: RC_BF16, torch.float16: RC_F16}
 _LIB = torch.library.Library("realcam", "DEF")
@@ -463,7 +463,7 @@
     b, H, W, _ = x.shape
     if out_mode == RC_OUT_NHWC:
         out = x.new_empty((b, H, W, cout))
-    elif out_mode == RC_OUT_PIXEL_SHUFFLE2:
+    elif out_mode in (RC_OUT_PIXEL_SHUFFLE2, RC_OUT_NHWC_IDWT):
         out = x.new_empty((b, 2 * H, 2 * W, cout // 4))
     elif out_mode == RC_OUT_NHWC_DWT:
         out = x.new_empty((b, H // 2, W // 2, 4 * cout))
```

New measurement: 1337 MP/s (median of 6 runs). About the same (+0.5%).
